# romz-pl/linear-programming-Vanderbei

Hardware: AMD Instinct MI355X
Metric: IPM iterations/sec (ADA^T factor+solve) on netlib dfl001; duality gap ≤1e-8 (higher is better)
Workload: dtype f64; 1 GPU; dfl001 hsd (BASELINE configs[2]), one step = one complete solve to mu < 1e-12; method=hsd, m=12155, n=12230, nz=71277, parallelism=replicas1, status=optimal solution, lnz=7160813, nsup=18147, levels=20, refine_passes=251

## Files before the change

### linear-programming-vanderbei_amd/csrc/dev_common.h

```cpp
#pragma once
#include <hip/hip_runtime.h>

#include <vector>

#include "row_ax.h"

namespace ipo {

constexpr int kRedBlocks = 256;
constexpr int kRedThreads = 256;

__device__ __forceinline__ double ref_max(double x, double y) { return x > y ? x : y; }
__device__ __forceinline__ double ref_abs(double x) { return x > 0 ? x : -x; }

template <int N>
__device__ __forceinline__ double dpp_row_down(double v) {
    const long long b = __double_as_longlong(v);
    const int lo = (int)b, hi = (int)(b >> 32);
    const int lo2 = __builtin_amdgcn_update_dpp(lo, lo, 0x100 + N, 0xf, 0xf, false);
    const int hi2 = __builtin_amdgcn_update_dpp(hi, hi, 0x100 + N, 0xf, 0xf, false);
    return __longlong_as_double(((long long)hi2 << 32) | (unsigned int)lo2);
}

__device__ __forceinline__ double wave_sum(double v) {
    v += __shfl_down(v, 32, 64);
    v += __shfl_down(v, 16, 64);
    v += dpp_row_down<8>(v);
    v += dpp_row_down<4>(v);
    v += dpp_row_down<2>(v);
    v += dpp_row_down<1>(v);
    return v;
}
__device__ __forceinline__ double wave_max(double v) {
    v = fmax(v, __shfl_down(v, 32, 64));
    v = fmax(v, __shfl_down(v, 16, 64));
    v = fmax(v, dpp_row_down<8>(v));
    v = fmax(v, dpp_row_down<4>(v));
    v = fmax(v, dpp_row_down<2>(v));
    v = fmax(v, dpp_row_down<1>(v));
    return v;
}

__device__ __forceinline__ double sparse_dot(int kb, int ke, const double* __restrict__ v, const int* __restrict__ idx,
                                             const double* __restrict__ x) {
    double s = 0.0;
    int k = kb;
    for (; k + 16 <= ke; k += 16) {
        int ix[16];
        double a[16], b[16];
#pragma unroll
        for (int u = 0; u < 16; u++) { ix[u] = idx[k + u]; a[u] = v[k + u]; }
#pragma unroll
        for (int u = 0; u < 16; u++) b[u] = x[ix[u]];
#pragma unroll
        for (int u = 0; u < 16; u++) s += a[u] * b[u];
    }
    const int rem = ke - k;
    if (rem > 0) {
        int ix[16];
        double a[16], b[16];
#pragma unroll
        for (int u = 0; u < 16; u++)
            if (u < rem) { ix[u] = idx[k + u]; a[u] = v[k + u]; }
#pragma unroll
        for (int u = 0; u < 16; u++)
            if (u < rem) b[u] = x[ix[u]];
#pragma unroll
        for (int u = 0; u < 16; u++)
            if (u < rem) s += a[u] * b[u];
    }
    return s;
}

template <int NW>
__device__ __forceinline__ double block_sum_w(double v, double* sh ) {
    v = wave_sum(v);
    const int lane = threadIdx.x & 63, w = threadIdx.x >> 6;
    if (lane == 0) sh[w] = v;
    __syncthreads();
    double r = 0.0;
    if (threadIdx.x == 0) {
        r = sh[0];
#pragma unroll
        for (int q = 1; q < NW; q++) r += sh[q];
    }
    __syncthreads();
    return r;
}
template <int NW>
__device__ __forceinline__ double block_max_w(double v, double* sh) {
    v = wave_max(v);
    const int lane = threadIdx.x & 63, w = threadIdx.x >> 6;
    if (lane == 0) sh[w] = v;
    __syncthreads();
    double r = 0.0;
    if (threadIdx.x == 0) {
        r = sh[0];
#pragma unroll
        for (int q = 1; q < NW; q++) r = fmax(r, sh[q]);
    }
    __syncthreads();
    return r;
}
constexpr int kResThreads = 1024;

__device__ __forceinline__ double block_sum(double v, double* sh ) {
    v = wave_sum(v);
    const int lane = threadIdx.x & 63, w = threadIdx.x >> 6;
    if (lane == 0) sh[w] = v;
    __syncthreads();
    double r = 0.0;
    if (threadIdx.x == 0) r = (sh[0] + sh[1]) + (sh[2] + sh[3]);
    __syncthreads();
    return r;
}
__device__ __forceinline__ double block_max(double v, double* sh) {
    v = wave_max(v);
    const int lane = threadIdx.x & 63, w = threadIdx.x >> 6;
    if (lane == 0) sh[w] = v;
    __syncthreads();
    double r = 0.0;
    if (threadIdx.x == 0) r = fmax(fmax(sh[0], sh[1]), fmax(sh[2], sh[3]));
    __syncthreads();
    return r;
}

__global__ void __launch_bounds__(kRedThreads)
k_finish_reduce(const double* __restrict__ part, int nq, unsigned maxmask, double* __restrict__ out);
__global__ void __launch_bounds__(kRedThreads)
k_finish_reduce_pack(const double* __restrict__ part, int nq, unsigned maxmask, double* __restrict__ out,
                     const int* __restrict__ f, int nf, double* __restrict__ outi);

struct RedJobs {
    const double* a[8];
    const double* b[8];
    int len[8];
    int op[8];
    int nj;
    int segmin;
};
__global__ void __launch_bounds__(kRedThreads)
k_reduce_jobs(RedJobs jobs, double* __restrict__ part);

constexpr int kOrderedMaxLen = 1 << 19;
constexpr int kSegDotLen = 1 << 12;
constexpr int kSegMaxLen = 1 << 16;
__host__ __device__ inline int dot_segmin(const RedJobs& j) { return j.segmin > 0 ? j.segmin : kOrderedMaxLen; }
__host__ __device__ inline bool job_segmented(const RedJobs& j, int q) {
    return j.len[q] >= (j.op[q] == 0 ? dot_segmin(j) : kSegMaxLen);
}
extern bool g_ordered_reductions;
void launch_reduce(const RedJobs& jobs, double* part, double* out, hipStream_t st);
double dot_ordered_host(const double* a, const double* b, int n);

void launch_link_ax(int mrow, int m, const int* kAt, const int* iAt, const double* At, const double* x, double* out,
                    hipStream_t st);

void launch_q_long(int nl, const int* cols, const int* kQ, const int* iQ, const double* Q, const double* v,
                   double* out, hipStream_t st);
__host__ __device__ inline bool q_col_long(const int* kQ, int j, int thr) {
    return thr > 0 && kQ[j + 1] - kQ[j] >= thr;
}
std::vector<int> q_long_columns(int n, const int* kQ, int thr);
void q_times_host(int n, const int* kQ, const int* iQ, const double* Q, const double* v, int thr, double* out);

}
```

### linear-programming-vanderbei_amd/csrc/dev_common.hip

```cpp
#include "dev_common.h"

#include <algorithm>
#include <cstdlib>
#include <stdexcept>
#include <vector>
#include "hip_util.h"

namespace ipo {

__global__ void __launch_bounds__(kRedThreads)
k_reduce_jobs(RedJobs jobs, double* __restrict__ part) {
    __shared__ double sh[4];
    for (int j = 0; j < jobs.nj; j++) {
        const double* a = jobs.a[j];
        const double* b = jobs.b[j];
        const int len = jobs.len[j];
        const int op = jobs.op[j];
        double acc = op == 0 ? 0.0 : (op == 2 ? 0.0 : 0.0);
        for (int i = blockIdx.x * kRedThreads + threadIdx.x; i < len; i += kRedBlocks * kRedThreads) {
            if (op == 0) acc += a[i] * b[i];
            else if (op == 1) acc = fmax(acc, ref_abs(a[i]));
            else acc = fmax(acc, -a[i] / b[i]);
        }
        const double r = op == 0 ? block_sum(acc, sh) : block_max(acc, sh);
        if (threadIdx.x == 0) part[j * kRedBlocks + blockIdx.x] = r;
    }
}

__global__ void __launch_bounds__(kRedThreads)
k_finish_reduce(const double* __restrict__ part, int nq, unsigned maxmask, double* __restrict__ out) {
    __shared__ double sh[4];
    for (int q = 0; q < nq; q++) {
        const bool mx = (maxmask >> q) & 1u;
        double v = part[q * kRedBlocks + threadIdx.x];
        const double r = mx ? block_max(v, sh) : block_sum(v, sh);
        if (threadIdx.x == 0) out[q] = r;
    }
}

__global__ void __launch_bounds__(kRedThreads)
k_finish_reduce_pack(const double* __restrict__ part, int nq, unsigned maxmask, double* __restrict__ out,
                     const int* __restrict__ f, int nf, double* __restrict__ outi) {
    __shared__ double sh[4];
    for (int q = 0; q < nq; q++) {
        const bool mx = (maxmask >> q) & 1u;
        double v = part[q * kRedBlocks + threadIdx.x];
        const double r = mx ? block_max(v, sh) : block_sum(v, sh);
        if (threadIdx.x == 0) out[q] = r;
    }
    if (static_cast<int>(threadIdx.x) < nf) reinterpret_cast<int*>(outi)[threadIdx.x] = f[threadIdx.x];
}

constexpr int kOrdThreads = 256;

__global__ void __launch_bounds__(kOrdThreads)
k_reduce_ordered(RedJobs jobs, double* __restrict__ out) {
    const int j = blockIdx.x;
    const double* a = jobs.a[j];
    const double* b = jobs.b[j];
    const int len = jobs.len[j];
    const int op = jobs.op[j];
    const int tid = threadIdx.x;
    if (job_segmented(jobs, j)) return;
    if (op != 0) {
        __shared__ double sh[4];
        double acc = 0.0;
        for (int i0 = 0; i0 < len; i0 += 8 * kOrdThreads) {
            double va[8], vb[8];
#pragma unroll
            for (int u = 0; u < 8; u++) {
                const int i = i0 + u * kOrdThreads + tid;
                va[u] = i < len ? a[i] : 0.0;
                vb[u] = op == 2 && i < len ? b[i] : 1.0;
            }
#pragma unroll
            for (int u = 0; u < 8; u++) {
                if (i0 + u * kOrdThreads + tid >= len) continue;
                if (op == 1) acc = fmax(acc, ref_abs(va[u]));
                else acc = fmax(acc, -va[u] / vb[u]);
            }
        }
        acc = block_max(acc, sh);
        if (tid == 0) out[j] = acc;
        return;
    }
    constexpr int CH = 4096;
    __shared__ __attribute__((aligned(16))) double comp[2][CH + 16];
    __shared__ int nzc[2], ready[2], freed[2];
    if (tid < 2) {
        ready[tid] = 0;
        freed[tid] = 0;
    }
    __syncthreads();
    const int nch = (len + CH - 1) / CH, lane = tid & 63, wv = tid >> 6;
    if (wv == 1) {
        for (int k = 0; k < nch; k++) {
            const int buf = k & 1;
            if (k >= 2)
                while (__hip_atomic_load(&freed[buf], __ATOMIC_ACQUIRE, __HIP_MEMORY_SCOPE_WORKGROUP) < k - 1)
                    __builtin_amdgcn_s_sleep(1);
            const int base = k * CH, cnt = min(CH, len - base);
            int off = 0;
            for (int i0 = 0; i0 < cnt; i0 += 8 * 64) {
                double pa[8], pb[8];
#pragma unroll
                for (int u = 0; u < 8; u++) {
                    const int i = i0 + u * 64 + lane;
                    pa[u] = i < cnt ? a[base + i] : 0.0;
                    pb[u] = i < cnt ? b[base + i] : 0.0;
                }
#pragma unroll
                for (int u = 0; u < 8; u++) {
                    const double v = pa[u] * pb[u];
                    const bool nzf = i0 + u * 64 + lane < cnt && v != 0.0;
                    const unsigned long long m = __ballot(nzf);
                    if (nzf) comp[buf][off + __popcll(m & ((1ull << lane) - 1ull))] = v;
                    off += __popcll(m);
                }
            }
            if (lane == 0) {
                nzc[buf] = off;
                __hip_atomic_store(&ready[buf], k + 1, __ATOMIC_RELEASE, __HIP_MEMORY_SCOPE_WORKGROUP);
            }
        }
        return;
    }
    if (tid != 0) return;
    double s = 0.0e0;
    for (int k = 0; k < nch; k++) {
        const int buf = k & 1;
        while (__hip_atomic_load(&ready[buf], __ATOMIC_ACQUIRE, __HIP_MEMORY_SCOPE_WORKGROUP) < k + 1)
            __builtin_amdgcn_s_sleep(1);
        const int nz = nzc[buf];
        const double2* pp = reinterpret_cast<const double2*>(comp[buf]);
        double2 cur[8];
#pragma unroll
        for (int u = 0; u < 8; u++) cur[u] = pp[u];
        int i = 0;
        for (; i + 16 <= nz; i += 16) {
            double2 nxt[8];
#pragma unroll
            for (int u = 0; u < 8; u++) nxt[u] = pp[(i + 16) / 2 + u];
#pragma unroll
            for (int u = 0; u < 8; u++) { s += cur[u].x; s += cur[u].y; }
#pragma unroll
            for (int u = 0; u < 8; u++) cur[u] = nxt[u];
        }
        for (; i < nz; i++) s += comp[buf][i];
        __hip_atomic_store(&freed[buf], k + 1, __ATOMIC_RELEASE, __HIP_MEMORY_SCOPE_WORKGROUP);
    }
    out[j] = s;
}

double dot_ordered_host(const double* a, const double* b, int n) {
    DevBuf<double> da(std::max(1, n)), db(std::max(1, n)), dout(8), dpart(8 * kRedBlocks);
    IPO_HIP_CHECK(hipMemcpy(da.get(), a, n * sizeof(double), hipMemcpyHostToDevice));
    IPO_HIP_CHECK(hipMemcpy(db.get(), b, n * sizeof(double), hipMemcpyHostToDevice));
    RedJobs j{};
    j.nj = 1;
    j.a[0] = da.get(); j.b[0] = db.get(); j.len[0] = n; j.op[0] = 0;
    launch_reduce(j, dpart.get(), dout.get(), nullptr);
    double r = 0.0;
    IPO_HIP_CHECK(hipMemcpy(&r, dout.get(), sizeof(double), hipMemcpyDeviceToHost));
    return r;
}

__global__ void __launch_bounds__(kOrdThreads)
k_dot_segments(RedJobs jobs, double* __restrict__ part) {
    const int j = blockIdx.y, g = blockIdx.x, tid = threadIdx.x;
    const int len = jobs.len[j], op = jobs.op[j];
    if (!job_segmented(jobs, j)) return;
    const long seg = (static_cast<long>(len) + kRedBlocks - 1) / kRedBlocks;
    const long b = seg * g, e = min(static_cast<long>(len), b + seg);
    const double* a = jobs.a[j];
    const double* bb = jobs.b[j];
    __shared__ double sh[kOrdThreads];
    double acc = 0.0;
    for (long i0 = b; i0 < e; i0 += 8 * kOrdThreads) {
        double pa[8], pb[8];
#pragma unroll
        for (int u = 0; u < 8; u++) {
            const long i = i0 + u * kOrdThreads + tid;
            pa[u] = i < e ? a[i] : 0.0;
            pb[u] = i < e && op != 1 ? bb[i] : 1.0;
        }
#pragma unroll
        for (int u = 0; u < 8; u++) {
            if (i0 + u * kOrdThreads + tid >= e) continue;
            if (op == 0) acc += pa[u] * pb[u];
            else if (op == 1) acc = fmax(acc, ref_abs(pa[u]));
            else acc = fmax(acc, -pa[u] / pb[u]);
        }
    }
    sh[tid] = acc;
    __syncthreads();
    if (tid == 0) {
        double s = 0.0;
        for (int t = 0; t < kOrdThreads; t++) s = op == 0 ? s + sh[t] : fmax(s, sh[t]);
        part[j * kRedBlocks + g] = s;
    }
}

__global__ void __launch_bounds__(64)
k_dot_finish(RedJobs jobs, const double* __restrict__ part, double* __restrict__ out) {
    const int j = threadIdx.x;
    if (j >= jobs.nj || !job_segmented(jobs, j)) return;
    const bool mx = jobs.op[j] != 0;
    double s = 0.0;
    for (int g = 0; g < kRedBlocks; g++) s = mx ? fmax(s, part[j * kRedBlocks + g]) : s + part[j * kRedBlocks + g];
    out[j] = s;
}

__global__ void __launch_bounds__(256)
k_link_ax(int mrow, int m, const int* __restrict__ kAt, const int* __restrict__ iAt, const double* __restrict__ At,
          const double* __restrict__ x, double* __restrict__ out) {
    const int i = mrow + blockIdx.x * 4 + (threadIdx.x >> 6), lane = threadIdx.x & 63;
    if (i >= m) return;
    double s = 0.0;
    for (int k = kAt[i] + lane; k < kAt[i + 1]; k += 64) s += At[k] * x[iAt[k]];
    s = wave_sum(s);
    if (lane == 0) out[i - mrow] = s;
}

void launch_link_ax(int mrow, int m, const int* kAt, const int* iAt, const double* At, const double* x, double* out,
                    hipStream_t st) {
    if (m <= mrow) return;
    hipLaunchKernelGGL(k_link_ax, dim3((m - mrow + 3) / 4), dim3(256), 0, st, mrow, m, kAt, iAt, At, x, out);
    IPO_HIP_CHECK(hipGetLastError());
}

constexpr int kQLongSteps = 4;

__global__ void __launch_bounds__(256)
k_q_long(int nl, const int* __restrict__ cols, const int* __restrict__ kQ, const int* __restrict__ iQ,
// ... 106 lines not shown
        for (int u = 0; u < 8; u++)
            if (ok[u]) b[u] = x[c[u]];
#pragma unroll
        for (int u = 0; u < 8; u++)
            if (ok[u]) s += a[u] * b[u];
    }
    ax[i] = s;
}

bool rows_ax_sliced(const KktKnobs& knobs, int n) {
    if (knobs.ax_jds >= 0) return knobs.ax_jds != 0;
    return knobs.ax_blocks > 1 || static_cast<long>(n) * static_cast<long>(sizeof(double)) > kAxSliceBytes;
}

void RowAxPlan::build(int m, int n, const int* kA, const int* iA, const double* A, int npass, hipStream_t st) {
    m_ = m;
    np_ = std::max(1, npass);
    const int per = (n + np_ - 1) / np_;
    auto slice = [&](int j) { return per > 0 ? std::min(np_ - 1, j / per) : 0; };
    std::vector<int> cnt(static_cast<size_t>(np_) * m, 0);
    for (int j = 0; j < n; j++)
        for (int k = kA[j]; k < kA[j + 1]; k++) cnt[static_cast<size_t>(slice(j)) * m + iA[k]]++;
    std::vector<int> perm(static_cast<size_t>(np_) * m), rank(static_cast<size_t>(np_) * m), dptr, dlen;
    rows_.assign(np_, 0);
    nd_.assign(np_, 0);
    dbase_.assign(np_ + 1, 0);
    long nz = 0;
    for (int p = 0; p < np_; p++) {
        const int* c = cnt.data() + static_cast<size_t>(p) * m;
        int mx = 0;
        for (int i = 0; i < m; i++) mx = std::max(mx, c[i]);
        std::vector<int> bucket(mx + 2, 0);
        for (int i = 0; i < m; i++) bucket[mx - c[i] + 1]++;
        for (int v = 0; v <= mx; v++) bucket[v + 1] += bucket[v];
        int* pp = perm.data() + static_cast<size_t>(p) * m;
        int* rk = rank.data() + static_cast<size_t>(p) * m;
        for (int i = 0; i < m; i++) { const int r = bucket[mx - c[i]]++; pp[r] = i; rk[i] = r; }
        int active = 0;
        while (active < m && c[pp[active]] > 0) active++;
        rows_[p] = p == 0 ? m : active;
        nd_[p] = mx;
        for (int k = 0, len = active; k < mx; k++) {
            while (len > 0 && c[pp[len - 1]] <= k) len--;
            dptr.push_back(static_cast<int>(nz));
            dlen.push_back(len);
            nz += len;
        }
        dbase_[p + 1] = static_cast<int>(dptr.size());
    }
    if (nz > static_cast<long>(INT32_MAX)) throw std::length_error("row products: more than 2^31 entries");
    std::vector<int> cols(nz), fill(static_cast<size_t>(np_) * m, 0);
    std::vector<double> vals(nz);
    for (int j = 0; j < n; j++) {
        const int p = slice(j);
        for (int k = kA[j]; k < kA[j + 1]; k++) {
            const size_t pi = static_cast<size_t>(p) * m + iA[k];
            const int q = dptr[dbase_[p] + fill[pi]++] + rank[pi];
            cols[q] = j;
            vals[q] = A[k];
        }
    }
    perm_.upload(perm, st);
    dptr_.upload(dptr, st);
    dlen_.upload(dlen, st);
    cols_.upload(cols, st);
    vals_.upload(vals, st);
    IPO_HIP_CHECK(hipStreamSynchronize(st));
}

void RowAxPlan::launch(const double* x, double* ax, hipStream_t st) const {
    for (int p = 0; p < np_; p++) {
        if (rows_[p] <= 0) continue;
        hipLaunchKernelGGL(k_rows_ax_jds, dim3((rows_[p] + 255) / 256), dim3(256), 0, st, rows_[p],
                           perm_.get() + static_cast<size_t>(p) * m_, dptr_.get() + dbase_[p], dlen_.get() + dbase_[p],
                           nd_[p], cols_.get(), vals_.get(), x, p == 0 ? 1 : 0, ax);
    }
    IPO_HIP_CHECK(hipGetLastError());
}

bool g_ordered_reductions = true;

void launch_reduce(const RedJobs& jobs, double* part, double* out, hipStream_t st) {
    if (g_ordered_reductions) {
        hipLaunchKernelGGL(k_reduce_ordered, dim3(jobs.nj), dim3(kOrdThreads), 0, st, jobs, out);
        bool longdot = false;
        for (int j = 0; j < jobs.nj; j++) longdot |= job_segmented(jobs, j);
        if (longdot) {
            hipLaunchKernelGGL(k_dot_segments, dim3(kRedBlocks, jobs.nj), dim3(kOrdThreads), 0, st, jobs, part);
            hipLaunchKernelGGL(k_dot_finish, dim3(1), dim3(64), 0, st, jobs, part, out);
        }
        IPO_HIP_CHECK(hipGetLastError());
        return;
    }
    unsigned mask = 0;
    for (int j = 0; j < jobs.nj; j++) if (jobs.op[j] != 0) mask |= 1u << j;
    hipLaunchKernelGGL(k_reduce_jobs, dim3(kRedBlocks), dim3(kRedThreads), 0, st, jobs, part);
    hipLaunchKernelGGL(k_finish_reduce, dim3(1), dim3(kRedThreads), 0, st, part, jobs.nj, mask, out);
    IPO_HIP_CHECK(hipGetLastError());
}

}
```

### linear-programming-vanderbei_amd/csrc/ipm.h

```cpp
#pragma once
#include <hip/hip_runtime.h>

#include <cstdio>
#include <memory>

#include "exchange.h"
#include "hip_util.h"
#include "kkt_device.h"
#include "row_ax.h"

namespace ipo {

enum class Method { Hsd = 0, Intpt = 1, Hsdls = 2, Qp = 3, Pc = 4 };

struct IpmOptions {
    Method method = Method::Hsd;
    int max_iter = 200;
    FILE* trace = nullptr;
    bool timing = false;
};

struct IpmResult {
    int status = 5;
    int iters = 0;
    double t_setup_s = 0.0;
    double t_solve_s = 0.0;
    double final_mu = 0.0, final_pobj = 0.0, final_dobj = 0.0, final_pinf = 0.0, final_dinf = 0.0;
    double phi = 1.0, psi = 1.0;
    KktTimers kkt;
    long refine_passes = 0;
};

struct ShardSpec {
    int nforced = 0;
    Exchange* xch = nullptr;
    int m_global = 0, n_global = 0;
    long nz_global = 0;
};

constexpr int kIsRed = 0;
constexpr int kIsZx = 0, kIsWy = 1, kIsCx = 2, kIsBy = 3;
constexpr int kIsXqx = 4;
constexpr int kIsPhiMu = 6;
constexpr int kIsNorm2 = 8;
constexpr int kIsTheta = 11;
constexpr int kIsDphi = 12;
constexpr int kIsPhiNext = 14;
constexpr int kIsPcRatio = 16;
constexpr int kIsPcDots = 17;
constexpr int kIsPcMu = 23;
constexpr int kIsCount = 24;

void vector_bench(int m, int n, const int* kA, const int* iA, const double* A, int reps, double* out, double* bytes);

class IpmSolver {
  public:
    IpmSolver(int m, int n, const int* kA, const int* iA, const double* A, const double* b, const double* c,
              double f, hipStream_t stream = nullptr, const ShardSpec* shard = nullptr, const QBlock* q = nullptr);
    ~IpmSolver();
    int run(const IpmOptions& opt, IpmResult* res);
    void download(double* x, double* y, double* w, double* z) const;
    KktDevice& kkt() { return *kkt_; }
    double setup_seconds() const { return t_setup_; }

  private:
    int run_hsd(const IpmOptions& opt, IpmResult* res);
    int run_intpt(const IpmOptions& opt, IpmResult* res);
    int run_hsdls(const IpmOptions& opt, IpmResult* res);
    int run_qp(const IpmOptions& opt, IpmResult* res);
    template <bool SW>
    int run_pc(const IpmOptions& opt, IpmResult* res);
    void reduce(const struct RedJobs& j, int nout);
    void link_ax(const double* x);
    void xsum(double* d, size_t n, RedOp op) { if (xch_) xch_->allreduce(d, n, op, stream_); }
    const double* lax() const { return xch_ ? lax_.get() : axsliced_ ? ax_.get() : nullptr; }
    int mrow() const { return xch_ ? m_ - nforced_ : axsliced_ ? 0 : m_; }
    void row_ax(const double* x, hipStream_t st);
    const KktKnobs knobs_ = KktKnobs::from_env();
    bool axsliced_ = false;
    DevBuf<double> ax_;
    RowAxPlan axplan_;
    void print_dims(FILE* tr) const;

    int m_, n_;
    double f_;
    hipStream_t stream_;
    bool own_stream_ = false;
    double t_setup_ = 0.0;
    int nforced_ = 0;
    Exchange* xch_ = nullptr;
    int mcnt_ = 0;
    int mg_ = 0, ng_ = 0;
    int dot_segmin_ = 0;
    long nzg_ = 0;
    std::unique_ptr<KktDevice> kkt_;
    bool has_q_ = false, sharded_ = false;
    DevBuf<double> qx_;
    DevBuf<double> b_, c_, x_, y_, w_, z_;
    DevBuf<double> rho_, sig_, D_, E_, fx_, fy_, gx_, gy_, dx_, dy_, dz_, dw_;
    DevBuf<double> part_, part2_, scal_, lax_;
    hipStream_t side_ = nullptr;
    hipEvent_t ev_step_ = nullptr, ev_side_ = nullptr;
    double* hs_ = nullptr;
};

int ipm_solve_host(int m, int n, int nz, const int* iA, const int* kA, const double* A, const double* b,
                   const double* c, double f, double* x, double* y, double* w, double* z, const IpmOptions& opt,
                   IpmResult* res);

}
```

### linear-programming-vanderbei_amd/csrc/ipm_device.hip

```cpp
#include <hip/hip_runtime.h>

#include <chrono>
#include <cmath>
#include <cstdlib>
#include <cstring>
#include <exception>
#include <stdexcept>
#include <vector>

#include "dev_common.h"
#include "hip_util.h"
#include "ipm.h"
#include "lp_io.h"

namespace ipo {

namespace {

constexpr int NT = 256;

__global__ void __launch_bounds__(NT) k_fill(int n, double v, double* __restrict__ a) {
    const int i = blockIdx.x * NT + threadIdx.x;
    if (i < n) a[i] = v;
}

__global__ void __launch_bounds__(kResThreads)
k_hsd_residuals(int m, int n, const int* __restrict__ kAt, const int* __restrict__ iAt, const double* __restrict__ At,
                const int* __restrict__ kA, const int* __restrict__ iA, const double* __restrict__ A,
                const double* __restrict__ b, const double* __restrict__ c, const double* __restrict__ x,
                const double* __restrict__ y, const double* __restrict__ w, const double* __restrict__ z, double phi_h,
                double delta, double mu_h, double* __restrict__ E, double* __restrict__ D, double* __restrict__ fy,
                double* __restrict__ fx, double* __restrict__ gy, double* __restrict__ gx, double* __restrict__ part,
                int mrow, int mcnt, const double* __restrict__ lax, const double* __restrict__ phimu) {
    __shared__ double sh[kResThreads / 64];
    const double phi = phimu ? phimu[0] : phi_h;
    const double mu = phimu ? phimu[1] : mu_h;
    const bool wde = phimu == nullptr;
    double sr = 0.0, ss = 0.0;
    for (int i = blockIdx.x * kResThreads + threadIdx.x; i < m + n; i += kRedBlocks * kResThreads) {
        if (i < m) {
            double ax = 0.0;
            if (i >= mrow) ax = lax[i - mrow];
            else
                ax = sparse_dot(kAt[i], kAt[i + 1], At, iAt, x);
            const double r1 = ax - b[i] * phi + w[i];
            if (i < mcnt) sr += r1 * r1;
            const double rho = -(1 - delta) * r1 + w[i] - delta * mu / y[i];
            if (wde) E[i] = w[i] / y[i];
            fy[i] = rho;
            gy[i] = -b[i];
        } else {
            const int j = i - m;
            double aty = 0.0;
            aty = sparse_dot(kA[j], kA[j + 1], A, iA, y);
            const double s1 = -aty + c[j] * phi + z[j];
            ss += s1 * s1;
            const double sg = -(1 - delta) * s1 + z[j] - delta * mu / x[j];
            if (wde) D[j] = z[j] / x[j];
            fx[j] = -sg;
            gx[j] = -c[j];
        }
    }
    sr = block_sum_w<kResThreads / 64>(sr, sh);
    ss = block_sum_w<kResThreads / 64>(ss, sh);
    if (threadIdx.x == 0) { part[blockIdx.x] = sr; part[kRedBlocks + blockIdx.x] = ss; }
}

__global__ void __launch_bounds__(NT)
k_hsd_directions(int m, int n, const double* __restrict__ dphip, double delta, double mu, const double* __restrict__ fx,
                 const double* __restrict__ gx, const double* __restrict__ fy, const double* __restrict__ gy,
                 const double* __restrict__ x, const double* __restrict__ z, const double* __restrict__ y,
                 const double* __restrict__ w, const double* __restrict__ D, const double* __restrict__ E,
                 double* __restrict__ dx, double* __restrict__ dz, double* __restrict__ dy, double* __restrict__ dw,
                 double* __restrict__ part) {
    __shared__ double sh[4];
    const double dphi = *dphip;
    double th = 0.0;
    for (int i = blockIdx.x * NT + threadIdx.x; i < m + n; i += kRedBlocks * NT) {
        if (i < n) {
            const double ddx = fx[i] - gx[i] * dphi;
            const double ddz = delta * mu / x[i] - z[i] - D[i] * ddx;
            dx[i] = ddx; dz[i] = ddz;
            th = fmax(th, -ddx / x[i]);
            th = fmax(th, -ddz / z[i]);
        } else {
            const int j = i - n;
            const double ddy = fy[j] - gy[j] * dphi;
            const double ddw = delta * mu / y[j] - w[j] - E[j] * ddy;
            dy[j] = ddy; dw[j] = ddw;
            th = fmax(th, -ddy / y[j]);
            th = fmax(th, -ddw / w[j]);
        }
    }
    th = block_max(th, sh);
    if (threadIdx.x == 0) part[blockIdx.x] = th;
}

__global__ void __launch_bounds__(NT)
k_step(int m, int n, double theta_h, const double* __restrict__ thetap, double* __restrict__ x,
       const double* __restrict__ dx, double* __restrict__ z, const double* __restrict__ dz, double* __restrict__ y,
       const double* __restrict__ dy, double* __restrict__ w, const double* __restrict__ dw) {
    const double theta = thetap ? *thetap : theta_h;
    const int i = blockIdx.x * NT + threadIdx.x;
    if (i < n) { x[i] = x[i] + theta * dx[i]; z[i] = z[i] + theta * dz[i]; }
    else if (i < n + m) { const int j = i - n; y[j] = y[j] + theta * dy[j]; w[j] = w[j] + theta * dw[j]; }
}

__global__ void __launch_bounds__(NT)
k_hsd_scaling(int m, int n, const double* __restrict__ x, const double* __restrict__ y, const double* __restrict__ w,
              const double* __restrict__ z, double* __restrict__ E, double* __restrict__ D) {
    const int i = blockIdx.x * NT + threadIdx.x;
    if (i < m) E[i] = w[i] / y[i];
    else if (i < m + n) { const int j = i - m; D[j] = z[j] / x[j]; }
}

__global__ void k_hsd_mu(double* sc, double denom, double phi_h, double psi_h, int dev) {
    const double phi = dev ? sc[kIsPhiNext] : phi_h, psi = dev ? sc[kIsPhiNext + 1] : psi_h;
    sc[kIsPhiMu] = phi;
    sc[kIsPhiMu + 1] = (sc[kIsZx] + sc[kIsWy] + phi * psi) / denom;
}

__global__ void k_hsd_dphi(double* sc, double gamma, double delta, double mu, double phi, double psi) {
    const double* red = sc + kIsRed;
    const double dphi = (red[0] - red[1] + gamma) / (red[2] - red[3] - psi / phi);
    const double dpsi = delta * mu / phi - psi - (psi / phi) * dphi;
    sc[kIsDphi] = dphi;
    sc[kIsDphi + 1] = dpsi;
}

__global__ void k_hsd_theta(double* sc, double phi, double psi) {
    const double dphi = sc[kIsDphi], dpsi = sc[kIsDphi + 1];
    double theta = sc[kIsRed];
    if (theta < -dphi / phi) theta = -dphi / phi;
    if (theta < -dpsi / psi) theta = -dpsi / psi;
    theta = (0.95 / theta > 1.0) ? 1.0 : 0.95 / theta;
    sc[kIsTheta] = theta;
    sc[kIsPhiNext] = phi + theta * dphi;
    sc[kIsPhiNext + 1] = psi + theta * dpsi;
}

__global__ void __launch_bounds__(NT)
k_unscale(int m, int n, double phi, double* __restrict__ x, double* __restrict__ z, double* __restrict__ y,
          double* __restrict__ w) {
    const int i = blockIdx.x * NT + threadIdx.x;
    if (i < n) { x[i] /= phi; z[i] /= phi; }
    else if (i < n + m) { const int j = i - n; y[j] /= phi; w[j] /= phi; }
}

__device__ __forceinline__ double ls_step(double xj, double zj, double dxj, double dzj, double beta, double delta,
                                          double mu) {
    const double a = dxj * dzj;
    const double b = zj * dxj + xj * dzj + (1 - beta) * (1 - delta) * mu;
    const double c = xj * zj - (1 - beta) * mu;
    const double d = b * b - 4 * a * c;
    if (a == 0.0) return -c / b;
    if (a > 0) {
        if (b < 0) {
            if (d >= 0) return 2 * c / (-b + sqrt(d));
            return HUGE_VAL;
        }
        return HUGE_VAL;
    }
    if (b < 0) return 2 * c / (-b + sqrt(d));
    return (-b - sqrt(d)) / (2 * a);
}

__global__ void __launch_bounds__(NT)
k_hsdls_directions(int m, int n, double dphi, double beta, double delta, double mu, const double* __restrict__ fx,
                   const double* __restrict__ gx, const double* __restrict__ fy, const double* __restrict__ gy,
                   const double* __restrict__ x, const double* __restrict__ z, const double* __restrict__ y,
                   const double* __restrict__ w, const double* __restrict__ D, const double* __restrict__ E,
                   double* __restrict__ dx, double* __restrict__ dz, double* __restrict__ dy, double* __restrict__ dw,
                   double* __restrict__ part) {
    __shared__ double sh[4];
    double th = -HUGE_VAL;
    for (int i = blockIdx.x * NT + threadIdx.x; i < m + n; i += kRedBlocks * NT) {
        if (i < n) {
            const double ddx = fx[i] - gx[i] * dphi;
            const double ddz = delta * mu / x[i] - z[i] - D[i] * ddx;
            dx[i] = ddx; dz[i] = ddz;
            th = fmax(th, -ls_step(x[i], z[i], ddx, ddz, beta, delta, mu));
        } else {
            const int j = i - n;
            const double ddy = fy[j] - gy[j] * dphi;
            const double ddw = delta * mu / y[j] - w[j] - E[j] * ddy;
            dy[j] = ddy; dw[j] = ddw;
            th = fmax(th, -ls_step(y[j], w[j], ddy, ddw, beta, delta, mu));
        }
    }
    th = block_max(th, sh);
    if (threadIdx.x == 0) part[blockIdx.x] = th;
}

__global__ void __launch_bounds__(kResThreads)
k_pf_residuals(int m, int n, const int* __restrict__ kAt, const int* __restrict__ iAt, const double* __restrict__ At,
               const int* __restrict__ kA, const int* __restrict__ iA, const double* __restrict__ A,
               const double* __restrict__ b, const double* __restrict__ c, const double* __restrict__ x,
               const double* __restrict__ y, const double* __restrict__ w, const double* __restrict__ z,
               double* __restrict__ rho, double* __restrict__ sig, double* __restrict__ part, int mrow, int mcnt,
               const double* __restrict__ lax) {
    __shared__ double sh[kResThreads / 64];
    double sr = 0.0, ss = 0.0;
    for (int i = blockIdx.x * kResThreads + threadIdx.x; i < m + n; i += kRedBlocks * kResThreads) {
        if (i < m) {
            double ax = 0.0;
            if (i >= mrow) ax = lax[i - mrow];
            else
                ax = sparse_dot(kAt[i], kAt[i + 1], At, iAt, x);
            const double r = b[i] - ax - w[i];
            rho[i] = r;
            if (i < mcnt) sr += r * r;
        } else {
            const int j = i - m;
            double aty = 0.0;
            aty = sparse_dot(kA[j], kA[j + 1], A, iA, y);
            const double s = c[j] - aty + z[j];
            sig[j] = s;
            ss += s * s;
        }
    }
    sr = block_sum_w<kResThreads / 64>(sr, sh);
// ... 208 lines not shown
    const double a = dxj * dzj;
    const double b = zj * dxj + xj * dzj + (1 - beta) * (1 - delta) * mu;
    const double c = xj * zj - (1 - beta) * mu;
    const double d = b * b - 4 * a * c;
    if (a == 0.0) return -c / b;
    if (a > 0) return (b < 0 && d >= 0) ? 2 * c / (-b + std::sqrt(d)) : HUGE_VAL;
    if (b < 0) return 2 * c / (-b + std::sqrt(d));
    return (-b - std::sqrt(d)) / (2 * a);
}

double now_s() {
    return std::chrono::duration<double>(std::chrono::steady_clock::now().time_since_epoch()).count();
}

const char* kHsdHeader =
    "--------------------------------------------------------------------------\n"
    "         |           Primal          |            Dual           |       |\n"
    "  Iter   |  Obj Value       Infeas   |  Obj Value       Infeas   |  mu   |\n"
    "- - - - - - - - - - - - - - - - - - - - - - - - - - - - - - - - - - - - - \n";
const char* kIntptHeader =
    "------------------------------------------------------------------\n"
    "         |           Primal          |            Dual           |\n"
    "  Iter   |  Obj Value       Infeas   |  Obj Value       Infeas   |\n"
    "- - - - - - - - - - - - - - - - - - - - - - - - - - - - - - - - - \n";

}

IpmSolver::IpmSolver(int m, int n, const int* kA, const int* iA, const double* A, const double* b, const double* c,
                     double f, hipStream_t stream, const ShardSpec* shard, const QBlock* q)
    : m_(m), n_(n), f_(f), stream_(stream) {
    const double t0 = now_s();
    sharded_ = shard != nullptr;
    has_q_ = q && q->kQ && q->kQ[n] > 0;
    if (has_q_ && sharded_) throw std::invalid_argument("qp: a solver with Q cannot be sharded");
    mg_ = m;
    ng_ = n;
    nzg_ = kA[n];
    mcnt_ = m;
    if (shard) {
        if (shard->nforced < 0 || shard->nforced > m) throw std::invalid_argument("shard: nforced out of range");
        nforced_ = shard->nforced;
        xch_ = shard->xch;
        if (xch_) {
            mg_ = shard->m_global;
            ng_ = shard->n_global;
            nzg_ = shard->nz_global;
            if (xch_->rank() != 0) mcnt_ = m - nforced_;
        }
    }
    dot_segmin_ = knobs_.dot_segmin >= 0 ? knobs_.dot_segmin : std::max(mg_, ng_) >= kOrderedMaxLen ? kSegDotLen : 0;
    if (!stream_) {
        IPO_HIP_CHECK(hipStreamCreateWithFlags(&stream_, hipStreamNonBlocking));
        own_stream_ = true;
    }
    if (has_q_) {
        std::vector<int> kat, iat;
        std::vector<double> at;
        csc_transpose(m, n, kA, iA, A, kat, iat, at);
        QBlock qb = *q;
        qb.qmax = 1;
        kkt_ = std::make_unique<KktDevice>(n, m, kat.data(), iat.data(), at.data(), stream_, 0, &qb);
    } else {
        kkt_ = std::make_unique<KktDevice>(m, n, kA, iA, A, stream_, nforced_);
        kkt_->set_exchange(xch_);
    }
    if (dot_segmin_ > 0 && !xch_ && !has_q_) {
        constexpr int kLongRow = 256;
        std::vector<int> cnt(m > 0 ? m : 1, 0);
        for (int k = 0; k < kA[n]; k++) cnt[iA[k]]++;
        int r0 = m;
        while (r0 > 0 && cnt[r0 - 1] >= kLongRow) r0--;
        if (r0 < m) kkt_->set_long_rows(r0);
    }
    const size_t mm = m > 0 ? m : 1, nn = n > 0 ? n : 1;
    b_.upload(b, m, stream_);
    c_.upload(c, n, stream_);
    for (DevBuf<double>* v : {&x_, &z_, &sig_, &D_, &fx_, &gx_, &dx_, &dz_, &qx_}) v->alloc(nn);
    for (DevBuf<double>* v : {&y_, &w_, &rho_, &E_, &fy_, &gy_, &dy_, &dw_}) v->alloc(mm);
    if (m == 0) b_.alloc(1);
    if (n == 0) c_.alloc(1);
    part_.alloc(8 * kRedBlocks);
    part2_.alloc(8 * kRedBlocks);
    scal_.alloc(kIsCount);
    IPO_HIP_CHECK(hipStreamCreateWithFlags(&side_, hipStreamNonBlocking));
    IPO_HIP_CHECK(hipEventCreateWithFlags(&ev_step_, hipEventDisableTiming));
    IPO_HIP_CHECK(hipEventCreateWithFlags(&ev_side_, hipEventDisableTiming));
    lax_.alloc(nforced_ > 0 ? nforced_ : 1);
    axsliced_ = rows_ax_sliced(knobs_, n_) && !xch_;
    if (axsliced_) {
        ax_.alloc(m_ > 0 ? m_ : 1);
        axplan_.build(m, n, kA, iA, A, knobs_.ax_blocks, stream_);
    }
    IPO_HIP_CHECK(hipHostMalloc(reinterpret_cast<void**>(&hs_), kIsCount * sizeof(double), hipHostMallocDefault));
    IPO_HIP_CHECK(hipStreamSynchronize(stream_));
    t_setup_ = now_s() - t0;
}

IpmSolver::~IpmSolver() {
    if (side_) (void)hipStreamSynchronize(side_);
    if (hs_) (void)hipHostFree(hs_);
    if (ev_step_) (void)hipEventDestroy(ev_step_);
    if (ev_side_) (void)hipEventDestroy(ev_side_);
    if (side_) (void)hipStreamDestroy(side_);
    kkt_.reset();
    if (own_stream_) (void)hipStreamDestroy(stream_);
}

void IpmSolver::reduce(const RedJobs& j, int nout) {
    launch_reduce(j, part_.get(), scal_.get(), stream_);
    xsum(scal_.get(), nout, RedOp::Sum);
    IPO_HIP_CHECK(hipMemcpyAsync(hs_, scal_.get(), nout * sizeof(double), hipMemcpyDeviceToHost, stream_));
    IPO_HIP_CHECK(hipStreamSynchronize(stream_));
}

void IpmSolver::row_ax(const double* x, hipStream_t st) {
    if (!axsliced_) return;
    axplan_.launch(x, ax_.get(), st);
}

void IpmSolver::link_ax(const double* x) {
    row_ax(x, stream_);
    if (!xch_ || nforced_ == 0) return;
    launch_link_ax(m_ - nforced_, m_, kkt_->kAt(), kkt_->iAt(), kkt_->At(), x, lax_.get(), stream_);
    xsum(lax_.get(), nforced_, RedOp::Sum);
}

void IpmSolver::print_dims(FILE* tr) const { std::fprintf(tr, "m = %d,n = %d,nz = %ld\n", mg_, ng_, nzg_); }

void IpmSolver::download(double* x, double* y, double* w, double* z) const {
    if (x) x_.download(x, n_, stream_);
    if (y) y_.download(y, m_, stream_);
    if (w) w_.download(w, m_, stream_);
    if (z) z_.download(z, n_, stream_);
    IPO_HIP_CHECK(hipStreamSynchronize(stream_));
}

int IpmSolver::run(const IpmOptions& opt, IpmResult* res) {
    IpmResult local;
    if (!res) res = &local;
    *res = IpmResult();
    const bool qp = opt.method == Method::Qp;
    if (qp && sharded_) throw std::invalid_argument("qp: not supported on a sharded solver");
    const bool pc = opt.method == Method::Pc;
    if (pc && sharded_) throw std::invalid_argument("pc: not supported on a sharded solver");
    if (!qp && !pc && has_q_) throw std::invalid_argument("a solver built with Q runs method qp only (hsd, intpt and hsdls are LP methods)");
    KktDevice& K = *kkt_;
    res->t_setup_s = t_setup_;
    K.enable_timing(opt.timing);
    K.reset_timers();
    K.set_epsdiag(1.0e-14);
    const double t0 = now_s();
    const int st = qp                            ? (has_q_ ? run_qp(opt, res) : run_intpt(opt, res))
                   : pc                          ? (has_q_ ? run_pc<true>(opt, res) : run_pc<false>(opt, res))
                   : opt.method == Method::Intpt ? run_intpt(opt, res)
                   : opt.method == Method::Hsdls ? run_hsdls(opt, res)
                                                 : run_hsd(opt, res);
    res->t_solve_s = now_s() - t0;
    res->status = st;
    res->kkt = K.timers();
    return st;
}

int IpmSolver::run_hsd(const IpmOptions& opt, IpmResult* res) {
    const bool overlap = xch_ == nullptr && knobs_.overlap;
    const int m = m_, n = n_;
    hipStream_t s = stream_;
    const int gv = ceil_div(m + n, NT);
    FILE* tr = opt.trace;
    hipLaunchKernelGGL(k_fill, dim3(ceil_div(n, NT)), dim3(NT), 0, s, n, 1.0, x_.get());
    hipLaunchKernelGGL(k_fill, dim3(ceil_div(n, NT)), dim3(NT), 0, s, n, 1.0, z_.get());
    hipLaunchKernelGGL(k_fill, dim3(ceil_div(m, NT)), dim3(NT), 0, s, m, 1.0, w_.get());
    hipLaunchKernelGGL(k_fill, dim3(ceil_div(m, NT)), dim3(NT), 0, s, m, 1.0, y_.get());
    double phi = 1.0, psi = 1.0;
    if (tr) {
        print_dims(tr);
        std::fputs(kHsdHeader, tr);
        std::fflush(tr);
    }
    KktDevice& K = *kkt_;
    int status = 5, iter;
    for (iter = 0; iter < opt.max_iter; iter++) {
        RedJobs j{};
        j.nj = 4;
        j.segmin = dot_segmin_;
        j.a[0] = z_.get(); j.b[0] = x_.get(); j.len[0] = n; j.op[0] = 0;
        j.a[1] = w_.get(); j.b[1] = y_.get(); j.len[1] = mcnt_; j.op[1] = 0;
        j.a[2] = c_.get(); j.b[2] = x_.get(); j.len[2] = n; j.op[2] = 0;
        j.a[3] = b_.get(); j.b[3] = y_.get(); j.len[3] = mcnt_; j.op[3] = 0;
        const double delta = (iter % 2 == 0) ? 0.0 : 1.0;
        KktDevice::HostState spec{};
        std::exception_ptr spec_err;
        if (overlap) {
            IPO_HIP_CHECK(hipEventRecord(ev_step_, s));
            IPO_HIP_CHECK(hipStreamWaitEvent(side_, ev_step_, 0));
            launch_reduce(j, part2_.get(), scal_.get(), side_);
            hipLaunchKernelGGL(k_hsd_mu, dim3(1), dim3(1), 0, side_, scal_.get(), static_cast<double>(ng_ + mg_ + 1), phi,
                               psi, iter > 0 ? 1 : 0);
            row_ax(x_.get(), side_);
            hipLaunchKernelGGL(k_hsd_residuals, dim3(kRedBlocks), dim3(kResThreads), 0, side_, m, n, K.kAt(), K.iAt(),
                               K.At(), K.kA(), K.iA(), K.A(), b_.get(), c_.get(), x_.get(), y_.get(), w_.get(), z_.get(),
                               phi, delta, 0.0, E_.get(), D_.get(), fy_.get(), fx_.get(), gy_.get(), gx_.get(),
                               part2_.get(), mrow(), mcnt_, lax(), static_cast<const double*>(scal_.get() + kIsPhiMu));
            hipLaunchKernelGGL(k_finish_reduce, dim3(1), dim3(kRedThreads), 0, side_, part2_.get(), 2, 0u,
                               scal_.get() + kIsNorm2);
            IPO_HIP_CHECK(hipMemcpyAsync(hs_, scal_.get(), kIsCount * sizeof(double), hipMemcpyDeviceToHost, side_));
            IPO_HIP_CHECK(hipEventRecord(ev_side_, side_));
            hipLaunchKernelGGL(k_hsd_scaling, dim3(gv), dim3(NT), 0, s, m, n, x_.get(), y_.get(), w_.get(), z_.get(),
                               E_.get(), D_.get());
            spec = K.host_state();
            KktDevice::PrePass pre;
            pre.R = 2;
            pre.dfy[0] = fy_.get(); pre.dfx[0] = fx_.get();
            pre.dfy[1] = gy_.get(); pre.dfx[1] = gx_.get();
            pre.stream = side_;
            pre.ready = ev_side_;
            try {
                K.factor(E_.get(), D_.get(), &pre);
            } catch (...) {
                spec_err = std::current_exception();
            }
            IPO_HIP_CHECK(hipEventSynchronize(ev_side_));
        } else {
            launch_reduce(j, part_.get(), scal_.get(), s);
            xsum(scal_.get(), 4, RedOp::Sum);
            IPO_HIP_CHECK(hipMemcpyAsync(hs_, scal_.get(), 4 * sizeof(double), hipMemcpyDeviceToHost, s));
            if (iter > 0)
                IPO_HIP_CHECK(hipMemcpyAsync(hs_ + kIsPhiNext, scal_.get() + kIsPhiNext, 2 * sizeof(double),
                                             hipMemcpyDeviceToHost, s));
            IPO_HIP_CHECK(hipStreamSynchronize(s));
        }
        if (iter > 0) { phi = hs_[kIsPhiNext]; psi = hs_[kIsPhiNext + 1]; }
        const double mu = (hs_[kIsZx] + hs_[kIsWy] + phi * psi) / (ng_ + mg_ + 1);
        if (overlap && (std::memcmp(&mu, &hs_[kIsPhiMu + 1], sizeof mu) != 0 ||
                        std::memcmp(&phi, &hs_[kIsPhiMu], sizeof phi) != 0))
            throw std::runtime_error("hsd: device mu / phi differ from the host's");
        const double pobj = hs_[kIsCx], dobj = hs_[kIsBy];
        if (mu < 1.0e-12) {
            if (overlap) K.restore_host_state(spec);
            if (phi > psi) status = 0;
            else if (dobj < 0.0) status = 2;
            else if (pobj > 0.0) status = 4;
            else { if (tr) std::fprintf(tr, "Trouble in river city \n"); status = 4; }
            break;
        }
        if (!overlap) {
            link_ax(x_.get());
            hipLaunchKernelGGL(k_hsd_residuals, dim3(kRedBlocks), dim3(kResThreads), 0, s, m, n, K.kAt(), K.iAt(), K.At(),
                               K.kA(), K.iA(), K.A(), b_.get(), c_.get(), x_.get(), y_.get(), w_.get(), z_.get(), phi,
                               delta, mu, E_.get(), D_.get(), fy_.get(), fx_.get(), gy_.get(), gx_.get(), part_.get(),
                               mrow(), mcnt_, lax(), static_cast<const double*>(nullptr));
            hipLaunchKernelGGL(k_finish_reduce, dim3(1), dim3(kRedThreads), 0, s, part_.get(), 2, 0u, scal_.get());
            xsum(scal_.get(), 2, RedOp::Sum);
            IPO_HIP_CHECK(hipMemcpyAsync(hs_ + kIsNorm2, scal_.get() + kIsRed, 2 * sizeof(double),
                                         hipMemcpyDeviceToHost, s));
            K.factor(E_.get(), D_.get());
        } else {
            if (spec_err) std::rethrow_exception(spec_err);
            IPO_HIP_CHECK(hipStreamWaitEvent(s, ev_side_, 0));
        }
        const double gamma = -(1 - delta) * (dobj - pobj + psi) + psi - delta * mu / phi;

        const double normr = std::sqrt(hs_[kIsNorm2]) / phi;
        const double norms = std::sqrt(hs_[kIsNorm2 + 1]) / phi;
        if (tr) {
            std::fprintf(tr, "%8d   %14.7e  %8.1e    %14.7e  %8.1e  %8.1e \n", iter, pobj / phi + f_, normr,
                         dobj / phi + f_, norms, mu);
            std::fflush(tr);
        }
        res->final_mu = mu; res->final_pobj = pobj / phi + f_; res->final_dobj = dobj / phi + f_;
        res->final_pinf = normr; res->final_dinf = norms;
        if (knobs_.trace_full) {
            std::fprintf(stderr, "FT %d %.17g %.17g %.17g %.17g %.17g %.17g\n", iter, pobj, dobj, mu, phi, psi, normr);
            std::fprintf(stderr, "FT   ndep=%d eps=%.1e\n", K.ndep(), K.epsdiag());
        }
        K.solve2(E_.get(), D_.get(), fy_.get(), fx_.get(), gy_.get(), gx_.get());
        res->refine_passes += K.last_passes();

        RedJobs q{};
        q.nj = 4;
        q.segmin = dot_segmin_;
        q.a[0] = c_.get(); q.b[0] = fx_.get(); q.len[0] = n; q.op[0] = 0;
        q.a[1] = b_.get(); q.b[1] = fy_.get(); q.len[1] = mcnt_; q.op[1] = 0;
        q.a[2] = c_.get(); q.b[2] = gx_.get(); q.len[2] = n; q.op[2] = 0;
        q.a[3] = b_.get(); q.b[3] = gy_.get(); q.len[3] = mcnt_; q.op[3] = 0;
        launch_reduce(q, part_.get(), scal_.get(), s);
        xsum(scal_.get(), 4, RedOp::Sum);
        hipLaunchKernelGGL(k_hsd_dphi, dim3(1), dim3(1), 0, s, scal_.get(), gamma, delta, mu, phi, psi);
        hipLaunchKernelGGL(k_hsd_directions, dim3(kRedBlocks), dim3(NT), 0, s, m, n, scal_.get() + kIsDphi, delta, mu,
                           fx_.get(), gx_.get(), fy_.get(), gy_.get(), x_.get(), z_.get(), y_.get(), w_.get(), D_.get(),
                           E_.get(), dx_.get(), dz_.get(), dy_.get(), dw_.get(), part_.get());
        hipLaunchKernelGGL(k_finish_reduce, dim3(1), dim3(kRedThreads), 0, s, part_.get(), 1, 1u, scal_.get());
        xsum(scal_.get(), 1, RedOp::Max);
        hipLaunchKernelGGL(k_hsd_theta, dim3(1), dim3(1), 0, s, scal_.get(), phi, psi);
        hipLaunchKernelGGL(k_step, dim3(gv), dim3(NT), 0, s, m, n, 0.0, scal_.get() + kIsTheta, x_.get(), dx_.get(),
                           z_.get(), dz_.get(), y_.get(), dy_.get(), w_.get(), dw_.get());
    }
    hipLaunchKernelGGL(k_unscale, dim3(gv), dim3(NT), 0, s, m, n, phi, x_.get(), z_.get(), y_.get(), w_.get());
    IPO_HIP_CHECK(hipGetLastError());
    IPO_HIP_CHECK(hipStreamSynchronize(s));
    res->iters = iter;
    res->phi = phi;
    res->psi = psi;
    return status;
}

int IpmSolver::run_hsdls(const IpmOptions& opt, IpmResult* res) {
    const int m = m_, n = n_;
    hipStream_t s = stream_;
    const int gv = ceil_div(m + n, NT);
    FILE* tr = opt.trace;
    hipLaunchKernelGGL(k_fill, dim3(ceil_div(n, NT)), dim3(NT), 0, s, n, 1.0, x_.get());
    hipLaunchKernelGGL(k_fill, dim3(ceil_div(n, NT)), dim3(NT), 0, s, n, 1.0, z_.get());
    hipLaunchKernelGGL(k_fill, dim3(ceil_div(m, NT)), dim3(NT), 0, s, m, 1.0, w_.get());
    hipLaunchKernelGGL(k_fill, dim3(ceil_div(m, NT)), dim3(NT), 0, s, m, 1.0, y_.get());
    double phi = 1.0, psi = 1.0;
    if (tr) {
        print_dims(tr);
        std::fputs(kHsdHeader, tr);
        std::fflush(tr);
    }
    const double beta = 0.80, delta = 2 * (1 - beta);
    KktDevice& K = *kkt_;
    int status = 5, iter;
    for (iter = 0; iter < opt.max_iter; iter++) {
        RedJobs j{};
        j.nj = 4;
        j.segmin = dot_segmin_;
        j.a[0] = z_.get(); j.b[0] = x_.get(); j.len[0] = n; j.op[0] = 0;
        j.a[1] = w_.get(); j.b[1] = y_.get(); j.len[1] = mcnt_; j.op[1] = 0;
        j.a[2] = c_.get(); j.b[2] = x_.get(); j.len[2] = n; j.op[2] = 0;
        j.a[3] = b_.get(); j.b[3] = y_.get(); j.len[3] = mcnt_; j.op[3] = 0;
        reduce(j, 4);
        const double mu = (hs_[kIsZx] + hs_[kIsWy] + phi * psi) / (ng_ + mg_ + 1);
        const double pobj = hs_[kIsCx], dobj = hs_[kIsBy];
        if (mu < 1.0e-12) {
            if (phi > 1.0e-12) status = 0;
            else if (dobj < 0.0) status = 2;
            else if (pobj > 0.0) status = 4;
            else status = 7;
            break;
        }
        link_ax(x_.get());
        hipLaunchKernelGGL(k_hsd_residuals, dim3(kRedBlocks), dim3(kResThreads), 0, s, m, n, K.kAt(), K.iAt(), K.At(), K.kA(),
                           K.iA(), K.A(), b_.get(), c_.get(), x_.get(), y_.get(), w_.get(), z_.get(), phi, delta, mu,
                           E_.get(), D_.get(), fy_.get(), fx_.get(), gy_.get(), gx_.get(), part_.get(), mrow(), mcnt_,
                           lax(), static_cast<const double*>(nullptr));
        hipLaunchKernelGGL(k_finish_reduce, dim3(1), dim3(kRedThreads), 0, s, part_.get(), 2, 0u, scal_.get());
        xsum(scal_.get(), 2, RedOp::Sum);
        IPO_HIP_CHECK(hipMemcpyAsync(hs_, scal_.get(), 2 * sizeof(double), hipMemcpyDeviceToHost, s));
        IPO_HIP_CHECK(hipStreamSynchronize(s));
        const double normr = std::sqrt(hs_[kIsRed]) / phi;
        const double norms = std::sqrt(hs_[kIsRed + 1]) / phi;
        const double gamma = -(1 - delta) * (dobj - pobj + psi) + psi - delta * mu / phi;
        if (tr) {
            std::fprintf(tr, "%8d   %14.7e  %8.1e    %14.7e  %8.1e  %8.1e \n", iter, pobj / phi + f_, normr,
                         dobj / phi + f_, norms, mu);
            std::fflush(tr);
        }
        res->final_mu = mu; res->final_pobj = pobj / phi + f_; res->final_dobj = dobj / phi + f_;
        res->final_pinf = normr; res->final_dinf = norms;

        K.factor(E_.get(), D_.get());
        K.solve2(E_.get(), D_.get(), fy_.get(), fx_.get(), gy_.get(), gx_.get());
        res->refine_passes += K.last_passes();

        RedJobs q{};
        q.nj = 4;
        q.segmin = dot_segmin_;
        q.a[0] = c_.get(); q.b[0] = fx_.get(); q.len[0] = n; q.op[0] = 0;
        q.a[1] = b_.get(); q.b[1] = fy_.get(); q.len[1] = mcnt_; q.op[1] = 0;
        q.a[2] = c_.get(); q.b[2] = gx_.get(); q.len[2] = n; q.op[2] = 0;
        q.a[3] = b_.get(); q.b[3] = gy_.get(); q.len[3] = mcnt_; q.op[3] = 0;
        reduce(q, 4);
        const double dphi = (hs_[kIsRed] - hs_[kIsRed + 1] + gamma) / (hs_[kIsRed + 2] - hs_[kIsRed + 3] - psi / phi);
        const double dpsi = delta * mu / phi - psi - (psi / phi) * dphi;

        hipLaunchKernelGGL(k_hsdls_directions, dim3(kRedBlocks), dim3(NT), 0, s, m, n, dphi, beta, delta, mu, fx_.get(),
                           gx_.get(), fy_.get(), gy_.get(), x_.get(), z_.get(), y_.get(), w_.get(), D_.get(), E_.get(),
// ... 369 lines not shown
```

### linear-programming-vanderbei_amd/csrc/kkt_device.h

```cpp
#pragma once
#include <hip/hip_runtime.h>

#include <cstddef>
#include <cstdint>
#include <memory>
#include <vector>

#include "hip_util.h"
#include "exchange.h"
#include "kkt_flags.h"
#include "kkt_knobs.h"
#include "kkt_plan.h"
#include "kkt_schedule.h"

namespace ipo {

struct TailView {
    double* S;
    int nt, ntb, tc;
    const int* task_ptr;
    const TailTask* tasks;
    double* W;
    int vk = kTailVisitBlocks;
    int dep = 1;
// ... 33 lines not shown
static_assert(RunCounters::vseq_at(3) == 4 && RunCounters::pread_at(3) == 13 && RunCounters::cdone_at(3) == 16 &&
                  RunCounters::lead_ticket_at(3) == 19 && RunCounters::words(3) == 20,
              "run counters, ntb = 3: 1 + 3 + 9 + 3 + 3 + 1");

constexpr int kTailPubWin = 16 * 64 + 16;

struct ChainGran {
    static constexpr size_t kZ = 2 * 64 * 2;
    static constexpr size_t kPart = 2 * 4 * 64 * 2;
    static constexpr size_t part_at(size_t ntb) { return ntb * kZ; }
    static constexpr size_t words(size_t ntb) { return ntb * (kZ + kPart); }
};

struct KktTimers {
    double phase_ms[kNumPhases] = {};
    long phase_launches[kNumPhases] = {};
    long phase_count[kNumPhases] = {};
    double factor_ms = 0.0;
    double solve_ms = 0.0;
    double sweep_ms = 0.0;
    long factors = 0, solves = 0, rawsolves = 0;
    long panel_redos = 0;
    long redo_where[4] = {0, 0, 0, 0};
    long tail_repairs = 0;
    long tail_dep_rounds = 0;
};

constexpr int kScRes = 0;
constexpr int kScEps = 4;
constexpr int kScIncons = 6;
constexpr int kScReadLater = kScIncons + 1;
constexpr int kScMaxbc = 8;
constexpr int kScCount = kScMaxbc + 4;
constexpr int kFsNegMinD = 0;
constexpr int kFsNdepMax = 1;
constexpr int kFsBailMax = 2;
constexpr int kFsFlags = 3;
constexpr int kFsCount = kFsFlags + 2;

struct QBlock {
    const int* kQ = nullptr;
    const int* iQ = nullptr;
    const double* Q = nullptr;
    int qmax = 1;
};

struct PlanView;

class KktDevice {
  public:
    KktDevice(int m, int n, const int* kA, const int* iA, const double* A, hipStream_t stream, int nforced = 0,
              const QBlock* qb = nullptr);
    ~KktDevice();
    KktDevice(const KktDevice&) = delete;
    KktDevice& operator=(const KktDevice&) = delete;

    const KktPlan& plan() const { return plan_; }
    void set_exchange(Exchange* x) { xch_ = x; }
    int nforced() const { return nforced_; }
    int m() const { return m_; }
    int n() const { return n_; }
    hipStream_t stream() const { return stream_; }

    const int* kA() const { return dkA_.get(); }
    const int* iA() const { return diA_.get(); }
    const double* A() const { return dA_.get(); }
    const int* kAt() const { return dkAt_.get(); }
    const int* iAt() const { return diAt_.get(); }
    const double* At() const { return dAt_.get(); }
    const int* kQ() const { return qnz_ > 0 ? dkQ_.get() : nullptr; }
    const int* iQ() const { return qnz_ > 0 ? diQ_.get() : nullptr; }
    const double* Q() const { return qnz_ > 0 ? dQ_.get() : nullptr; }
    int q_long_count() const { return q_long_n_; }
    int q_long_min() const { return q_long_n_ > 0 ? knobs_.q_long : 0; }
    void launch_q_long(const double* v, double* out);

    struct PrePass {
        int R = 0;
        double* dfy[2] = {nullptr, nullptr};
        double* dfx[2] = {nullptr, nullptr};
        hipStream_t stream = nullptr;
        hipEvent_t ready = nullptr;
    };
    void factor(const double* dE, const double* dD, const PrePass* pre = nullptr);
    int solve(const double* dE, const double* dD, double* dfy, double* dfx);
    int solve2(const double* dE, const double* dD, double* dfy1, double* dfx1, double* dfy2, double* dfx2);
    void solve_multi(int R, const double* dE, const double* dD, double* const* dfy, double* const* dfx, int* ok);

    void rawsolve(double* dz, int R = 1, size_t fwd_first = 0);

    struct HostState {
        double epsdiag;
        int ndep;
        KktTimers tm;
    };
    HostState host_state() const { return {epsdiag_, ndep_, tm_}; }
    void restore_host_state(const HostState& h) { epsdiag_ = h.epsdiag; ndep_ = h.ndep; tm_ = h.tm; drop_prepass(); }

    double epsdiag() const { return epsdiag_; }
    void set_pivot_tolerance(double t) { pivot_tol_ = t; }
    void set_epsdiag(double e) { epsdiag_ = e; }
    void set_long_rows(int row0);
    double pivot_tolerance() const { return pivot_tol_; }
    int ndep() const { return ndep_; }
    int last_passes() const { return last_passes_; }
    const KktTimers& timers() const { return tm_; }
    void enable_timing(bool on) { timing_ = on; }
    void reset_timers() { tm_ = KktTimers(); }

    void download_factor(double* lx, double* d, int* live = nullptr) const;
    double* device_lx() const { return dLx_.get(); }
    double* device_diag() const { return dDg_.get(); }

  private:
    const KktKnobs knobs_ = KktKnobs::from_env();
    void upload_plan(const int* kA, const int* iA, const double* A, const std::vector<int>& kat,
                     const std::vector<int>& iat, const std::vector<double>& at, const QBlock* qb);
    void build_panel_units();
    SolveChunks build_solve_chunks();
    SweepOrder build_sweep_order(const SolveChunks& ch);
    void build_sync_free_plan(const SolveChunks& ch, const SweepOrder& so, int cus);
    void build_gather_chunks(const VisitSlots& vs);
    void count_work();
    void build_slot_records(const std::vector<int>& kslot_v);
    void setup_tail(int cus);
    void alloc_numeric();
    void raise_sweep_lds(bool sync_free);
    void dump_sf_stamps() const;
    KktLaunch h_;
    PlanView plan_view() const;
    bool tail_repair() const { return use_panel_ && !xch_ && knobs_.tail_repair; }
    void factor_core(const double* dE, const double* dD, const PrePass* pre);
    void dump_factor(const double* dE, const double* dD, double eps_in);
    int dump_count_ = 0;
    TailView tail_view() const;
    template <int R>
    void sweep(double* dz, const double* epsp, size_t fwd_first);
    template <int R>
    int run_sweep_steps(const std::vector<SweepStep>& steps, bool forward, double* dz, const double* epsp,
                        size_t first = 0, size_t last = SIZE_MAX, hipStream_t s = nullptr);
    void tail_rhs_begin(double* dz, int R);
    void tail_rhs_end(double* dz, int R);
    DevBuf<int> dIncons_;
    int launch_gather(const struct PlanView& pv, const TailView& tv, int tail, int group, hipStream_t s);
    void launch_reduce_maxabs2(const double* a, int na, const double* b, int nb, double* dst);

    int m_, n_, T_;
    int nforced_ = 0;
    Exchange* xch_ = nullptr;
    DevBuf<double> dLinkAx_;
    int long_row0_ = -1;
    DevBuf<double> dLongAx_;
    bool shard_minor() const { return xch_ && xch_->rank() != 0; }
    void xsum(double* d, size_t n, RedOp op) { if (xch_) xch_->allreduce(d, n, op, stream_); }
    hipStream_t stream_;
    KktPlan plan_;
    double epsdiag_ = 1.0e-14;
    int ndep_ = 0;
    double pivot_tol_ = knobs_.pivtol;
    int last_passes_ = 0;
    bool timing_ = false;
    KktTimers tm_;
    hipEvent_t ev0_ = nullptr, ev1_ = nullptr, ev2_ = nullptr, ev3_ = nullptr;
    std::vector<hipEvent_t> kev_;
    size_t kev_used_ = 0;
    struct PhaseMark { hipEvent_t b, e; int phase, launches; };
    std::vector<PhaseMark> marks_;
    hipEvent_t mark_b_ = nullptr;
    hipEvent_t next_event();
    void ph_begin(hipStream_t s);
    void ph_end(int phase, int launches, hipStream_t s);
    void ph_collect();
  public:
    double work_flops[kNumPhases] = {}, work_bytes[kNumPhases] = {};
  private:

    DevBuf<int> dkA_, diA_, dkAt_, diAt_;
    DevBuf<double> dA_, dAt_;
    int qnz_ = 0, qmax_ = 1;
    DevBuf<int> dkQ_, diQ_;
    DevBuf<double> dQ_, dQdiag_;
    DevBuf<int64_t> dqmap_;
    int q_long_n_ = 0;
    DevBuf<int> dQLongCols_;
    DevBuf<double> dLongQ_;
    DevBuf<int> dcol0_, drowptr_, drows_, dperm_, diperm_;
    DevBuf<int64_t> doff_, damap_, ddslot_, drelptr_;
    DevBuf<int> dunit_sup_, dunit_tile_, dtask_ptr_, dtask_pair_, dtask_i0_, dtask_i1_;
    DevBuf<int> dupd_src_, dupd_r0_, dupd_r1_, drel_, dlevel_sups_;
    DevBuf<int> dyrow_ptr_, dyrow_idx_;
    DevBuf<int> dylate_ptr_, dylate_idx_, dpre_col_, dpre_ptr_, dpre_idx_;
    DevBuf<double> dYbuf_;
    int sf_grid_ = 1;
    int sf_fwd_epoch_ = 0, sf_bwd_epoch_ = 0;
    long long sf_ticket_next_[2] = {0, 0};
#ifdef IPO_SF_STAMPS
    std::vector<SchedInt2> h_sf_items_f_;
#endif
    int sf_tbase(int d, int nitems, hipStream_t s);
    DevBuf<int2> dsf_items_f_, dsf_items_b_;
    DevBuf<int> dsf_need_, dsf_par_, dsf_zbase_, dsf_zpi_, dsf_fcnt_, dsf_fflag_, dsf_bcnt_, dsf_bflag_, dsf_ticket_;
    DevBuf<int> dybase_;
    DevBuf<double> dZpad_;
    DevBuf<int> dfu_sup_, dfu_j_;
    DevBuf<int> dsmall_sups_;
    const bool use_panel_ = knobs_.panel;
    bool factor_pass(const double* dE, const double* dD, bool fused, bool tail_fused, const PrePass* pre = nullptr);
    bool prepass_eligible(const PrePass* pre, bool fused, bool tail_fused) const;
    void enqueue_prepass(const PrePass& pre);
    void run_prepass_steps(int R, hipStream_t q);
    void enqueue_pass_head(int R, double* const* dfy, double* const* dfx, double* part, hipStream_t s);
    bool take_prepass(int R, double* const* dfy, double* const* dfx);
    void drop_prepass() {
        if (pre_state_ != kPreNone) { pre_state_ = kPreNone; pre_discarded_++; lead_discarded_ += pre_lead_; }
        pre_lead_ = false;
        lead_pending_ = 0;
    }
    enum { kPreNone = 0, kPreEnqueued, kPreValid };
    int pre_state_ = kPreNone;
    PrePass pre_req_;
    hipEvent_t ev_pre_fork_ = nullptr, ev_pre_done_ = nullptr;
    long pre_used_ = 0, pre_discarded_ = 0;
    int lead_pending_ = 0;
    bool pre_lead_ = false;
    hipEvent_t ev_run_reset_ = nullptr;
    long lead_used_ = 0, lead_discarded_ = 0;
    void launch_lead_trail(int R, hipStream_t s, bool beside);
    DevBuf<double> dPrePart_;
    void enqueue_levels(const PlanView& pv, const TailView& tv, bool fused, hipStream_t s, const PrePass* pre);
    bool finish_pass(bool fused);
    void repair_tail();
    DevBuf<int> dsweep_sups_;
    DevBuf<int> dchunk_sup_, dchunk_r0_, dsup_chunk0_;
    DevBuf<double> dPartial_;
    int gst_group_ = knobs_.gather_stamps, gst_n_ = 0;
    DevBuf<long long> dGStamp_;
    DevBuf<int> dck_u_, dck_b_, dck_e_, dck_part_, dsp_u_, dsp_p0_, dsp_n_;
    DevBuf<int> dck_q_;
    DevBuf<int> dSplitCnt_;
    bool eps_cleared_ = false;
    DevBuf<double> dPartialTile_;
    DevBuf<TaskSrc> dusrc_, dtsrc_;
    DevBuf<SlotRec> dslot_rec_, dtail_slot_rec_;
    DevBuf<unsigned long long> dChainGran_;
    int chain_epoch_ = 0;
    DevBuf<int> dtail_task_ptr_, dtail_kslot_, dtail_kslot_ptr_;
    DevBuf<int> dlead_ticket_;
    long long lead_ticket_next_ = 0;
    DevBuf<unsigned> dvisit_list_;
    DevBuf<uint2> drun_items_;
    DevBuf<int> drun_cnt_;
    RunCounters run_counters() const { return RunCounters(drun_cnt_.get(), plan_.ntb); }
    DevBuf<double> drun_pub_;
    DevBuf<int> drun_wflag_;
    int run_epoch_ = 0;
    void launch_tail_from(int t0, bool reset);
    DevBuf<uint64_t> dtail_tasks_, dutasks_;
    DevBuf<double> dW_;
    DevBuf<double> dDepSt_;
    DevBuf<int> dDepI_;
    DevBuf<double> dLx_, dDg_;
    DevBuf<int> dLive_;
    DevBuf<double> dDscale_;
    DevBuf<int> dFlags_;
    DevBuf<int> dSign_;
    DevBuf<double> dZ_, dDy_, dDx_, dRy_, dRx_;
    DevBuf<double> dPart_;
    DevBuf<double> dScal_;
    double* sweep_eps() const { return dScal_.get() + kScEps; }
    DevBuf<double> dFacScal_;
    double* hScal_ = nullptr;
    int* hDepDone_ = nullptr;
    FactorVerdict verdict_;
};

}
```

### linear-programming-vanderbei_amd/csrc/kkt_device.hip

```cpp
#include <hip/hip_runtime.h>

#include <chrono>
#include <algorithm>
#include <cmath>
#include <cstdio>
#include <cstdlib>
#include <cstring>

#include "dev_common.h"
#include "kkt_device.h"
#include "kkt_kernels.h"
#include "lp_io.h"

namespace ipo {

namespace {

__global__ void __launch_bounds__(NT)
k_assemble_A(int nz, const double* __restrict__ A, const int64_t* __restrict__ amap, double* __restrict__ Lx) {
    const int k = blockIdx.x * NT + threadIdx.x;
    if (k < nz) Lx[amap[k]] = A[k];
}

__global__ void __launch_bounds__(NT)
k_assemble_Q(int nq, const double* __restrict__ Q, const int64_t* __restrict__ qmap, double qmax,
             double* __restrict__ Lx) {
    const int k = blockIdx.x * NT + threadIdx.x;
    if (k < nq && qmap[k] >= 0) Lx[qmap[k]] = -qmax * Q[k];
}

__global__ void __launch_bounds__(NT)
k_assemble_diag(int T, int m, const int* __restrict__ perm, const double* __restrict__ E,
                const double* __restrict__ D, double eps, const int64_t* __restrict__ dslot,
                double* __restrict__ Lx, int* __restrict__ live, double* __restrict__ dscale, int tail_from,
                int* __restrict__ flags, const double* __restrict__ qdiag, double qmax) {
    const int v = blockIdx.x * NT + threadIdx.x;
    if (v < kFlagWords) flags[v] = 0;
    if (v >= T) return;
    const int old = perm[v];
    double a = v >= tail_from ? 0.0 : old < m ? -ref_max(E[old], eps) : ref_max(D[old - m], eps);
    double sc = fabs(a);
    if (qdiag && old < m) {
        const double q = qmax * qdiag[old];
        a = a - q;
        sc = sc + fabs(q);
    }
    Lx[dslot[v]] = a;
    dscale[v] = sc;
    live[v] = 1;
}

__global__ void __launch_bounds__(NT) k_zero_tail_lower(double* __restrict__ S, int nt) {
    const int c = blockIdx.x;
    double* col = S + (size_t)c * nt;
    for (int r = (c / kPanelCols) * kPanelCols + static_cast<int>(threadIdx.x); r < nt; r += NT) col[r] = 0.0;
}

typedef double double4_t __attribute__((ext_vector_type(4)));
constexpr int KS = kSlab;

struct SlotLd {
    double a, b, d;
    bool ra, rb;
};
__device__ __forceinline__ SlotLd slot_ld(const SlotRec& m, const double* __restrict__ Lx,
                                          const double* __restrict__ dg, int lane) {
    const uint64_t below = (1ull << lane) - 1ull;
    SlotLd v;
    v.ra = (m.rmask >> lane) & 1ull;
    v.rb = (m.cmask >> lane) & 1ull;
    v.a = Lx[v.ra ? m.roff + __popcll(m.rmask & below) : m.roff];
    v.b = Lx[v.rb ? m.roff + m.cdelta + __popcll(m.cmask & below) : m.roff];
    v.d = dg[m.dk];
    return v;
}
__device__ __forceinline__ void slot_fin(const SlotLd& v, double& ra, double& rb) {
    ra = v.ra ? v.a : 0.0;
    rb = v.rb ? v.d * v.b : 0.0;
}

struct GatherTile {
    double* out;
    size_t ld;
    int nrow, ncol, row0, col0;
    double* dscale_col;
};

__device__ __forceinline__ GatherTile unit_tile(const PlanView& p, const TailView& tv, int u, int tail) {
    GatherTile g;
    if (tail < 0) {
        const int s = p.unit_sup[u], t = p.unit_tile[u];
        const int c0 = p.col0[s], nc = p.col0[s + 1] - c0;
        const int h = nc + (p.rowptr[s + 1] - p.rowptr[s]);
        const int rbase = t * TR;
        g.out = p.Lx + p.off[s] + rbase;
        g.ld = h;
        g.nrow = min(TR, h - rbase);
        g.ncol = nc;
        g.row0 = rbase;
        g.col0 = 0;
        g.dscale_col = t == 0 ? p.dscale + c0 : nullptr;
    } else {
        int bi = 0;
        while ((bi + 1) * (bi + 2) / 2 <= u) bi++;
        const int bj = u - bi * (bi + 1) / 2;
        g.out = tv.S + bi * TR + (size_t)(bj * TR) * tv.nt;
        g.ld = tv.nt;
        g.nrow = min(TR, tv.nt - bi * TR);
        g.ncol = min(TR, tv.nt - bj * TR);
        g.row0 = bi * TR;
        g.col0 = bj * TR;
        g.dscale_col = bi == bj ? p.dscale + tv.tc + bj * TR : nullptr;
    }
    return g;
}

__device__ void gather_acc(const PlanView& p, const SlotRec* __restrict__ recs, int kb, int ke, int dcol,
                           bool has_diag, double4_t (&acc)[2][2], double& dabs) {
    __shared__ double As[2][TR][KS + 1];
    __shared__ double Bs[2][TR][KS + 1];
    const int tid = threadIdx.x;
    const int wv = __builtin_amdgcn_readfirstlane(tid >> 6), lane = tid & 63;
    const int wr = (wv & 1) * 32, wc = (wv >> 1) * 32;
    const int li = lane & 15, lk = lane >> 4;
#pragma unroll
    for (int a = 0; a < 2; a++)
#pragma unroll
        for (int b = 0; b < 2; b++) acc[a][b] = (double4_t){0.0, 0.0, 0.0, 0.0};
    dabs = 0.0;
    const int nk = ke - kb, nslab = nk / KS;
    double ra[KS / 4], rb[KS / 4];
    const double* __restrict__ Lx = p.Lx;
    const double* __restrict__ dg = p.dg;
    const SlotRec* __restrict__ wrec = recs + kb + wv * (KS / 4);
    SlotRec mn[KS / 4];
    auto fetch = [&](int slab) {
#pragma unroll
        for (int j = 0; j < KS / 4; j++) mn[j] = wrec[slab * KS + j];
// ... 427 lines not shown
    for (int kk = 0; kk < PC; kk += 4) {
        double av[2], bv[2];
        for (int a = 0; a < 2; a++) av[a] = As[wr + a * 16 + li][kk + lk];
        for (int b = 0; b < 2; b++) bv[b] = Bs[wc + b * 16 + li][kk + lk];
        for (int a = 0; a < 2; a++)
            for (int b = 0; b < 2; b++) acc[a][b] = __builtin_amdgcn_mfma_f64_16x16x4f64(av[a], bv[b], acc[a][b], 0, 0, 0);
    }
    const bool diag_tile = bi == bj;
    double old[2][2][4];
#pragma unroll
    for (int a = 0; a < 2; a++)
#pragma unroll
        for (int b = 0; b < 2; b++)
#pragma unroll
            for (int i = 0; i < 4; i++) {
                const int rr = wr + a * 16 + (lane >> 4) + 4 * i;
                const int cc = wc + b * 16 + (lane & 15);
                const int rg = bi * TR + rr, cg = bj * TR + cc;
                const bool ok = rg < nt && cg < nt && !(diag_tile && cc > rr);
                old[a][b][i] = ok ? tv.S[rg + (size_t)cg * nt] : 0.0;
            }
#pragma unroll
    for (int a = 0; a < 2; a++)
#pragma unroll
        for (int b = 0; b < 2; b++)
#pragma unroll
            for (int i = 0; i < 4; i++) {
                const int rr = wr + a * 16 + (lane >> 4) + 4 * i;
                const int cc = wc + b * 16 + (lane & 15);
                const int rg = bi * TR + rr, cg = bj * TR + cc;
                if (rg >= nt || cg >= nt || (diag_tile && cc > rr)) continue;
                tv.S[rg + (size_t)cg * nt] = old[a][b][i] - acc[a][b][i];
            }
    if (diag_tile && tid < TR) {
        const int rg = bi * TR + tid;
        if (rg < nt) {
            double as = 0.0;
            for (int k = 0; k < nc; k++) as += fabs(As[tid][k] * Bs[tid][k]);
            p.dscale[tv.tc + rg] += as;
        }
    }
}

struct PermJobs {
    const double* fy[2];
    const double* fx[2];
    double* z[2];
    double* dy[2];
    double* dx[2];
    int mode[2];
};
__global__ void __launch_bounds__(NT)
k_perm_in2(int T, int m, const int* __restrict__ perm, PermJobs J, int* __restrict__ zi, double* __restrict__ zd) {
    const int v = blockIdx.x * NT + threadIdx.x, q = blockIdx.y;
    if (q == 0 && v < 2 && zi) { zi[v] = 0; zd[v] = 0.0; }
    if (v >= T) return;
    const int o = perm[v];
    J.z[q][v] = o < m ? J.fy[q][o] : J.fx[q][o - m];
}
__global__ void __launch_bounds__(NT)
k_perm_out2(int T, int m, const int* __restrict__ iperm, PermJobs J) {
    const int o = blockIdx.x * NT + threadIdx.x, q = blockIdx.y;
    if (o >= T) return;
    const double v = J.z[q][iperm[o]];
    double* dst = o < m ? J.dy[q] + o : J.dx[q] + (o - m);
    const int mode = J.mode[q];
    if (mode == 0) *dst = v;
    else if (mode == 1) *dst = *dst + v;
    else *dst = *dst - v;
}

__global__ void __launch_bounds__(NT)
k_perm_out(int T, int m, const int* __restrict__ iperm, const double* __restrict__ z, double* __restrict__ dy,
           double* __restrict__ dx, int mode) {
    const int o = blockIdx.x * NT + threadIdx.x;
    if (o >= T) return;
    const double v = z[iperm[o]];
    double* dst = o < m ? dy + o : dx + (o - m);
    if (mode == 0) *dst = v;
    else if (mode == 1) *dst = *dst + v;
    else *dst = *dst - v;
}

__device__ __forceinline__ void kkt_residual_body(
    int m, int n, const int* __restrict__ kAt, const int* __restrict__ iAt, const double* __restrict__ At,
    const int* __restrict__ kA, const int* __restrict__ iA, const double* __restrict__ A, const double* __restrict__ E,
    const double* __restrict__ D, const double* __restrict__ fy, const double* __restrict__ fx,
    const double* __restrict__ dy, const double* __restrict__ dx, double* __restrict__ ry, double* __restrict__ rx,
    double* __restrict__ part, int mrow, const double* __restrict__ axl, const int* __restrict__ kQ,
    const int* __restrict__ iQ, const double* __restrict__ Q, double qmax, int qthr,
    const double* __restrict__ qxl) {
    __shared__ double sh[kResThreads / 64];
    double mx = 0.0;
    for (int i = blockIdx.x * kResThreads + threadIdx.x; i < m + n; i += kRedBlocks * kResThreads) {
        if (i < m) {
            double s = 0.0;
            if (i >= mrow) s = axl[i - mrow];
            else
                s = sparse_dot(kAt[i], kAt[i + 1], At, iAt, dx);
            const double r = kQ ? fy[i] - ((s - E[i] * dy[i]) -
                                           qmax * (q_col_long(kQ, i, qthr) ? qxl[i]
                                                                           : sparse_dot(kQ[i], kQ[i + 1], Q, iQ, dy)))
                                : fy[i] - (s - E[i] * dy[i]);
            ry[i] = r;
            mx = fmax(mx, ref_abs(r));
        } else {
            const int j = i - m;
            double s = 0.0;
            s = sparse_dot(kA[j], kA[j + 1], A, iA, dy);
            const double r = fx[j] - (s + D[j] * dx[j]);
            rx[j] = r;
            mx = fmax(mx, ref_abs(r));
        }
    }
    mx = block_max_w<kResThreads / 64>(mx, sh);
    if (threadIdx.x == 0) part[blockIdx.x] = mx;
}


struct ResJobs {
    const double* fy[2];
    const double* fx[2];
    const double* dy[2];
    const double* dx[2];
    double* ry[2];
    double* rx[2];
    const double* axl[2];
    const double* qxl[2];
};
__global__ void __launch_bounds__(kResThreads)
k_kkt_residual2(int m, int n, const int* __restrict__ kAt, const int* __restrict__ iAt, const double* __restrict__ At,
                const int* __restrict__ kA, const int* __restrict__ iA, const double* __restrict__ A,
                const double* __restrict__ E, const double* __restrict__ D, ResJobs J, double* __restrict__ part,
                int mrow, const int* __restrict__ kQ, const int* __restrict__ iQ, const double* __restrict__ Q,
                double qmax, int qthr) {
    const int q = blockIdx.y;
    kkt_residual_body(m, n, kAt, iAt, At, kA, iA, A, E, D, J.fy[q], J.fx[q], J.dy[q], J.dx[q], J.ry[q], J.rx[q],
                      part + (size_t)q * kRedBlocks, mrow, J.axl[q], kQ, iQ, Q, qmax, qthr, J.qxl[q]);
}

__global__ void __launch_bounds__(NT)
k_min_abs_partial(const double* __restrict__ d, int T, double* __restrict__ part) {
    __shared__ double sh[4];
    double mn = HUGE_VAL;
    for (int i = blockIdx.x * NT + threadIdx.x; i < T; i += kRedBlocks * NT) mn = fmin(mn, ref_abs(d[i]));
    const double r = block_max(-mn, sh);
    if (threadIdx.x == 0) part[blockIdx.x] = r;
}

struct CopyOut {
    const double* src[4];
    double* dst[4];
    int m, n, R;
};
__global__ void __launch_bounds__(NT) k_copy_out(CopyOut c) {
    const int i = blockIdx.x * NT + threadIdx.x, per = c.m + c.n;
    if (i >= c.R * per) return;
    const int r = i / per, k = i - r * per;
    if (k < c.m) c.dst[2 * r][k] = c.src[2 * r][k];
    else c.dst[2 * r + 1][k - c.m] = c.src[2 * r + 1][k - c.m];
}
__global__ void k_pack_ints(const int* f, int n, double* out) {
    if (static_cast<int>(threadIdx.x) < n) reinterpret_cast<int*>(out)[threadIdx.x] = f[threadIdx.x];
}
__global__ void k_flag_to_scalar(const int* f, double* d) { d[0] = static_cast<double>(f[0]); }

}

KktDevice::KktDevice(int m, int n, const int* kA, const int* iA, const double* A, hipStream_t stream, int nforced,
                     const QBlock* qb)
    : m_(m), n_(n), T_(m + n), nforced_(nforced), stream_(stream) {
    if (qb && !qb->kQ) qb = nullptr;
    if (qb && nforced > 0) throw std::invalid_argument("kkt: a Q block with forced rows is not supported");
    QPattern qpat;
    if (qb) { qpat.kQ = qb->kQ; qpat.iQ = qb->iQ; }
    const auto st0 = std::chrono::steady_clock::now();
    auto mark = [&](const char* what) {
        if (knobs_.setup_times)
            std::fprintf(stderr, "setup %-28s %9.1f ms\n", what,
                         std::chrono::duration<double, std::milli>(std::chrono::steady_clock::now() - st0).count());
    };
    std::vector<int> kat, iat;
    std::vector<double> at;
    csc_transpose(m, n, kA, iA, A, kat, iat, at);
    const double tail_density = device_tail_density();
    mark("transpose");
    plan_ = build_kkt_plan(m, n, kA, iA, kat.data(), iat.data(), nforced, tail_density, qb ? &qpat : nullptr);
    mark("ordering + symbolic plan");
    h_.paths = kkt_paths(plan_, knobs_);
    int dev = 0, cus = 0;
    IPO_HIP_CHECK(hipGetDevice(&dev));
    IPO_HIP_CHECK(hipDeviceGetAttribute(&cus, hipDeviceAttributeMultiprocessorCount, dev));
    upload_plan(kA, iA, A, kat, iat, at, qb);
    mark("upload_plan");
    build_panel_units();
    mark("build_panel_units");
    {
        const SolveChunks ch = build_solve_chunks();
        mark("build_solve_chunks");
        const SweepOrder so = build_sweep_order(ch);
        mark("build_sweep_order");
        build_sync_free_plan(ch, so, cus);
        mark("build_sync_free_plan");
    }
    const VisitSlots vs = build_visit_slots(plan_, knobs_, h_.paths);
    mark("build_visit_slots");
    build_gather_chunks(vs);
    mark("build_gather_chunks");
    count_work();
    mark("count_work");
    build_slot_records(vs.kslot);
    mark("build_slot_records");
    setup_tail(cus);
    mark("setup_tail");
    alloc_numeric();
    mark("alloc_numeric");
}

void KktDevice::upload_plan(const int* kA, const int* iA, const double* A, const std::vector<int>& kat,
                            const std::vector<int>& iat, const std::vector<double>& at, const QBlock* qb) {
    const int m = m_, n = n_;
    if (nforced_ > 0) dLinkAx_.alloc(2 * static_cast<size_t>(nforced_));
    const int nz = kA[n];
    hipStream_t s = stream_;
    dkA_.upload(kA, n + 1, s);
    diA_.upload(iA, nz, s);
    dA_.upload(A, nz, s);
    dkAt_.upload(kat, s);
    diAt_.upload(iat, s);
    dAt_.upload(at, s);
// ... 112 lines not shown
    build(plan_.utasks, dusrc_);
    if (plan_.nt > 0) build(plan_.tail_tasks, dtsrc_);
    auto expand = [&](const std::vector<int>& kslot, const std::vector<TailTask>& ts, DevBuf<SlotRec>& dst) {
        const std::vector<SlotRec> v = ipo::build_slot_records(plan_, kslot, ts);
        dst.upload(v, s);
        IPO_HIP_CHECK(hipStreamSynchronize(s));
    };
    expand(h_.paths.visits ? kslot_v : plan_.kslot, plan_.utasks, dslot_rec_);
    if (plan_.nt > 0) expand(plan_.tail_kslot, plan_.tail_tasks, dtail_slot_rec_);
    dutasks_.upload(reinterpret_cast<const uint64_t*>(plan_.utasks.data()), plan_.utasks.size() * 4, s);
}

void KktDevice::setup_tail(int cus) {
    hipStream_t s = stream_;
    if (plan_.nt > 0) {
        dtail_task_ptr_.upload(plan_.tail_task_ptr, s);
        dtail_kslot_.upload(plan_.tail_kslot, s);
        dtail_kslot_ptr_.upload(plan_.tail_kslot_ptr, s);
        static_assert(sizeof(TailTask) == 32, "TailTask layout");
        dtail_tasks_.upload(reinterpret_cast<const uint64_t*>(plan_.tail_tasks.data()), plan_.tail_tasks.size() * 4, s);
        dW_.alloc(static_cast<size_t>(plan_.nt) * kPanelCols);
        dDepSt_.alloc(tail_dep_state_doubles(plan_.ntb));
        dDepI_.alloc(8);
        dChainGran_.alloc(ChainGran::words(plan_.ntb));
        dlead_ticket_.alloc(1);
        IPO_HIP_CHECK(hipMemsetAsync(dlead_ticket_.get(), 0, sizeof(int), s));
        lead_ticket_next_ = 0;
        IPO_HIP_CHECK(hipMemsetAsync(dChainGran_.get(), 0, dChainGran_.bytes(), s));
    }
    raise_sweep_lds(false);
    if (plan_.nt > 0 && plan_.ntb <= kTailSchedMaxBlocks) {
        TailSchedule ts = build_tail_schedule(plan_, knobs_, h_.paths, cus);
        if (knobs_.visit_sched) {
            dvisit_list_.upload(ts.visit_list, s);
            IPO_HIP_CHECK(hipStreamSynchronize(s));
            h_.visit_ptr = std::move(ts.visit_ptr);
        }
        if (h_.paths.tail_run) {
            static_assert(sizeof(SchedUint2) == sizeof(uint2), "SchedUint2 is uploaded as uint2");
            drun_items_.upload(reinterpret_cast<const uint2*>(ts.run_items.data()), ts.run_items.size(), s);
            h_.run_ptr = std::move(ts.run_ptr);
            drun_cnt_.alloc(RunCounters::words(plan_.ntb));
            if (h_.paths.run_winpub) {
                drun_pub_.alloc(2 * static_cast<size_t>(plan_.ntb) * 4 * kTailPubWin);
                drun_wflag_.alloc(static_cast<size_t>(plan_.ntb) * plan_.ntb * 4);
                IPO_HIP_CHECK(hipMemsetAsync(drun_wflag_.get(), 0, drun_wflag_.bytes(), s));
                run_epoch_ = 0;
            }
            IPO_HIP_CHECK(hipStreamSynchronize(s));
        }
    }
}

void KktDevice::alloc_numeric() {
    hipStream_t s = stream_;
    dLx_.alloc(plan_.lx_size > 0 ? plan_.lx_size : 1);
    dDg_.alloc(T_ > 0 ? T_ : 1);
    dLive_.alloc(T_ > 0 ? T_ : 1);
    dDscale_.alloc(T_ > 0 ? T_ : 1);
    dFlags_.alloc(kFlagWords);
    IPO_HIP_CHECK(hipMemsetAsync(dFlags_.get(), 0, dFlags_.bytes(), s));
    dSign_.upload(plan_.dsign, s);
    dZ_.alloc(2 * (T_ > 0 ? T_ : 1));
    dDy_.alloc(2 * (m_ > 0 ? m_ : 1));
    dRy_.alloc(2 * (m_ > 0 ? m_ : 1));
    dDx_.alloc(2 * (n_ > 0 ? n_ : 1));
    dRx_.alloc(2 * (n_ > 0 ? n_ : 1));
    dIncons_.alloc(2);
    dPart_.alloc(8 * kRedBlocks);
    dScal_.alloc(kScCount);
    dFacScal_.alloc(kFsCount);
    static_assert(kFlagReadWords * sizeof(int) <= (kFsCount - kFsFlags) * sizeof(double), "the packed flag words");
    dPrePart_.alloc(8 * kRedBlocks);
    IPO_HIP_CHECK(hipHostMalloc(reinterpret_cast<void**>(&hScal_), std::max(kScCount, kFsCount) * sizeof(double),
                                hipHostMallocDefault));
    IPO_HIP_CHECK(hipHostMalloc(reinterpret_cast<void**>(&hDepDone_), sizeof(int), hipHostMallocDefault));
    IPO_HIP_CHECK(hipEventCreate(&ev0_));
    IPO_HIP_CHECK(hipEventCreate(&ev1_));
    IPO_HIP_CHECK(hipEventCreate(&ev2_));
    IPO_HIP_CHECK(hipEventCreate(&ev3_));
    IPO_HIP_CHECK(hipEventCreateWithFlags(&ev_pre_fork_, hipEventDisableTiming));
    IPO_HIP_CHECK(hipEventCreateWithFlags(&ev_pre_done_, hipEventDisableTiming));
    IPO_HIP_CHECK(hipEventCreateWithFlags(&ev_run_reset_, hipEventDisableTiming));
    IPO_HIP_CHECK(hipStreamSynchronize(s));
}

void KktDevice::build_sync_free_plan(const SolveChunks& ch, const SweepOrder& so, int cus) {
    hipStream_t s = stream_;
    dyrow_ptr_.upload(plan_.yrow_ptr, s);
    const SyncFreePlan sf = ipo::build_sync_free_plan(plan_, knobs_, h_.paths, ch);
    const int ns = plan_.nsup;
    h_.sf_level = sf.sf_level;
    dyrow_idx_.upload(sf.yrow_idx, s);
    dybase_.upload(sf.ybase, s);
    if (sf.late_lists) {
        dylate_ptr_.upload(sf.ylate_ptr, s);
        dylate_idx_.upload(sf.ylate_idx.empty() ? std::vector<int>{0} : sf.ylate_idx, s);
        dpre_col_.upload(sf.pre_col.empty() ? std::vector<int>{0} : sf.pre_col, s);
        dpre_ptr_.upload(sf.pre_ptr, s);
        dpre_idx_.upload(sf.pre_idx.empty() ? std::vector<int>{0} : sf.pre_idx, s);
        IPO_HIP_CHECK(hipStreamSynchronize(s));
    }
    h_.ybuf_stride = sf.ybuf_stride;
    dYbuf_.alloc(2 * h_.ybuf_stride);
    h_.sweep = build_sweep_steps(plan_, knobs_, h_.paths, ch, so, sf, h_.paths.tail_blocked);
    if (sf.range(plan_)) {
        static_assert(sizeof(SchedInt2) == sizeof(int2), "SchedInt2 is uploaded as int2");
        dsf_items_f_.upload(reinterpret_cast<const int2*>(sf.items_f.data()), sf.items_f.size(), s);
#ifdef IPO_SF_STAMPS
        h_sf_items_f_ = sf.items_f;
#endif
        dsf_items_b_.upload(reinterpret_cast<const int2*>(sf.items_b.data()), sf.items_b.size(), s);
        dsf_need_.upload(sf.need, s);
        dsf_par_.upload(sf.par, s);
        dsf_zbase_.upload(sf.zbase, s);
        dsf_zpi_.upload(sf.zpi, s);
        h_.zpad_stride = sf.zpad_stride;
        dZpad_.alloc(2 * h_.zpad_stride);
        for (DevBuf<int>* b : {&dsf_fcnt_, &dsf_fflag_, &dsf_bcnt_, &dsf_bflag_}) {
            b->alloc(ns);
            IPO_HIP_CHECK(hipMemsetAsync(b->get(), 0, ns * sizeof(int), s));
        }
        dsf_ticket_.alloc(2);
        IPO_HIP_CHECK(hipMemsetAsync(dsf_ticket_.get(), 0, 2 * sizeof(int), s));
        sf_ticket_next_[0] = sf_ticket_next_[1] = 0;
        sf_grid_ = cus;
    }
    raise_sweep_lds(true);
    IPO_HIP_CHECK(hipStreamSynchronize(s));
}

KktDevice::~KktDevice() {
    dump_sf_stamps();
    if (knobs_.debug_redo)
        std::fprintf(stderr, "kkt: %ld factorisations, %ld redone; bails (unused) %ld, k_panel_w sparse %ld, tail %ld, "
                             "k_panel_s %ld; tail block columns repaired %ld in %ld rounds\n", tm_.factors,
                     tm_.panel_redos, tm_.redo_where[0], tm_.redo_where[1], tm_.redo_where[2], tm_.redo_where[3],
                     tm_.tail_repairs, tm_.tail_dep_rounds);
    if (knobs_.debug_redo) {
        std::fprintf(stderr, "kkt: forward pre-passes used %ld, discarded %ld\n", pre_used_, pre_discarded_);
        std::fprintf(stderr, "kkt: trailing leads used %ld, discarded %ld\n", lead_used_, lead_discarded_);
    }
    if (hScal_) (void)hipHostFree(hScal_);
    if (hDepDone_) (void)hipHostFree(hDepDone_);
    if (ev0_) (void)hipEventDestroy(ev0_);
    if (ev1_) (void)hipEventDestroy(ev1_);
    if (ev2_) (void)hipEventDestroy(ev2_);
    if (ev3_) (void)hipEventDestroy(ev3_);
    if (ev_pre_fork_) (void)hipEventDestroy(ev_pre_fork_);
    if (ev_pre_done_) (void)hipEventDestroy(ev_pre_done_);
    if (ev_run_reset_) (void)hipEventDestroy(ev_run_reset_);
    for (hipEvent_t e : kev_) (void)hipEventDestroy(e);
}

PlanView KktDevice::plan_view() const {
    PlanView v;
    v.col0 = dcol0_.get(); v.rowptr = drowptr_.get(); v.rows = drows_.get(); v.off = doff_.get();
    v.unit_sup = dunit_sup_.get(); v.unit_tile = dunit_tile_.get();
    v.task_ptr = dtask_ptr_.get(); v.task_pair = dtask_pair_.get();
    v.task_i0 = dtask_i0_.get(); v.task_i1 = dtask_i1_.get();
    v.upd_src = dupd_src_.get(); v.upd_r0 = dupd_r0_.get(); v.upd_r1 = dupd_r1_.get();
    v.relptr = drelptr_.get(); v.rel = drel_.get();
    v.Lx = dLx_.get(); v.dg = dDg_.get(); v.live = dLive_.get();
    v.flags = dFlags_.get();
    v.sign = dSign_.get();
    v.xcd = knobs_.update_xcd;
    v.dscale = dDscale_.get();
    v.tau = pivot_tol_;
    v.incons = dIncons_.get();
    v.ybase = dybase_.get();
    return v;
}

TailView KktDevice::tail_view() const {
    TailView t;
    t.S = dLx_.get() + plan_.off_tail;
    t.nt = plan_.nt;
    t.ntb = plan_.ntb;
    t.tc = plan_.tail_c0;
    t.task_ptr = dtail_task_ptr_.get();
    t.tasks = reinterpret_cast<const TailTask*>(dtail_tasks_.get());
    t.W = dW_.get();
    t.vk = knobs_.visit_blocks;
    if (!h_.visit_ptr.empty()) {
        t.vlist = dvisit_list_.get();
        t.vptr = h_.visit_ptr.data();
    }
    t.dep = tail_repair() ? knobs_.tail_spec : 0;
    t.sdep = knobs_.sparse_dep;
    return t;
}

void KktDevice::dump_factor(const double* dE, const double* dD, double eps_in) {
    if (knobs_.dump_dir.empty()) return;
    std::vector<double> E(m_), D(n_), dg(T_), dsc(T_);
    std::vector<int> live(T_);
    IPO_HIP_CHECK(hipStreamSynchronize(stream_));
    if (m_) IPO_HIP_CHECK(hipMemcpy(E.data(), dE, m_ * sizeof(double), hipMemcpyDeviceToHost));
    if (n_) IPO_HIP_CHECK(hipMemcpy(D.data(), dD, n_ * sizeof(double), hipMemcpyDeviceToHost));
    dLive_.download(live.data(), T_, stream_);
    dDg_.download(dg.data(), T_, stream_);
    dDscale_.download(dsc.data(), T_, stream_);
    IPO_HIP_CHECK(hipStreamSynchronize(stream_));
    char path[4096];
    std::snprintf(path, sizeof path, "%s/f%04d.bin", knobs_.dump_dir.c_str(), dump_count_++);
    FILE* f = std::fopen(path, "wb");
    if (!f) return;
    const int hdr[4] = {m_, n_, T_, ndep_};
    const double eps[2] = {eps_in, epsdiag_};
    std::fwrite(hdr, sizeof(int), 4, f);
    std::fwrite(eps, sizeof(double), 2, f);
    std::fwrite(E.data(), sizeof(double), m_, f);
    std::fwrite(D.data(), sizeof(double), n_, f);
    std::fwrite(plan_.perm.data(), sizeof(int), T_, f);
    std::fwrite(live.data(), sizeof(int), T_, f);
    std::fwrite(dg.data(), sizeof(double), T_, f);
    std::fwrite(dsc.data(), sizeof(double), T_, f);
    std::fclose(f);
}

void KktDevice::factor(const double* dE, const double* dD, const PrePass* pre) {
    const double eps_in = epsdiag_;
    drop_prepass();
    try {
        factor_core(dE, dD, pre);
    } catch (...) {
        if (pre_state_ != kPreNone) (void)hipStreamWaitEvent(stream_, ev_pre_done_, 0);
        drop_prepass();
        throw;
    }
    dump_factor(dE, dD, eps_in);
}

void KktDevice::factor_core(const double* dE, const double* dD, const PrePass* pre) {
    const bool repair = tail_repair();
    const bool ok = factor_pass(dE, dD, use_panel_, use_panel_, pre);
    if (!ok) {
        tm_.panel_redos++;
        for (int b = 0; b < 4; b++) tm_.redo_where[b] += (verdict_.bail >> b) & 1;
        if (repair && verdict_.tail_only()) repair_tail();
        else if (!factor_pass(dE, dD, false, repair) && repair && verdict_.tail_only()) repair_tail();
    }
    tm_.factors++;
    if (timing_)
        for (int ph : {kPhGather, kPhDiag, kPhTrsm, kPhSyrk, kPhTail}) tm_.phase_count[ph]++;
    ndep_ = verdict_.ndep_all;
    if (pre_state_ == kPreEnqueued) {
        if (ok && ndep_ == 0) pre_state_ = kPreValid;
        else drop_prepass();
    }
    if (verdict_.min_d < 1.0e-14) epsdiag_ *= 10;
    if (knobs_.epsdiag_max > 0.0 && epsdiag_ > knobs_.epsdiag_max) epsdiag_ = knobs_.epsdiag_max;
}

bool KktDevice::factor_pass(const double* dE, const double* dD, bool fused, bool tail_fused, const PrePass* pre) {
    hipStream_t s = stream_;
    if (timing_) IPO_HIP_CHECK(hipEventRecord(ev0_, s));
    const PlanView pv = plan_view();
    const int nz = static_cast<int>(plan_.amap.size());
    if (plan_.nt > 0 && !xch_) {
        if (plan_.off_tail > 0) IPO_HIP_CHECK(hipMemsetAsync(dLx_.get(), 0, plan_.off_tail * sizeof(double), s));
        hipLaunchKernelGGL(k_zero_tail_lower, dim3(plan_.nt), dim3(NT), 0, s, dLx_.get() + plan_.off_tail, plan_.nt);
    } else {
        IPO_HIP_CHECK(hipMemsetAsync(dLx_.get(), 0, dLx_.bytes(), s));
    }
    if (nz > 0) hipLaunchKernelGGL(k_assemble_A, dim3(ceil_div(nz, NT)), dim3(NT), 0, s, nz, dA_.get(), damap_.get(), dLx_.get());
    if (qnz_ > 0)
        hipLaunchKernelGGL(k_assemble_Q, dim3(ceil_div(qnz_, NT)), dim3(NT), 0, s, qnz_, dQ_.get(), dqmap_.get(),
                           static_cast<double>(qmax_), dLx_.get());
    hipLaunchKernelGGL(k_assemble_diag, dim3(ceil_div(T_, NT)), dim3(NT), 0, s, T_, m_, dperm_.get(), dE, dD, epsdiag_,
                       ddslot_.get(), dLx_.get(), dLive_.get(), dDscale_.get(), shard_minor() ? plan_.tail_c0 : T_,
                       dFlags_.get(), dkQ_.get() ? dQdiag_.get() : static_cast<const double*>(nullptr),
                       static_cast<double>(qmax_));
    const TailView tv = tail_view();
    if (!prepass_eligible(pre, fused, tail_fused)) pre = nullptr;
    enqueue_levels(pv, tv, fused, s, pre);
    if (plan_.nt > 0) {
        xsum(tv.S, static_cast<size_t>(plan_.nt) * plan_.nt, RedOp::Sum);
        xsum(dDscale_.get() + plan_.tail_c0, plan_.nt, RedOp::Sum);
        if (tail_fused && h_.paths.tail_run) {
            launch_tail_from(0, true);
        } else if (tail_fused) {
            ph_begin(s);
            for (int t = 0; t < plan_.ntb; t++) launch_tail_step(pv, tv, t, s);
            ph_end(kPhTail, plan_.ntb, s);
        } else
        for (int kb = 0; kb < plan_.ntb; kb++) {
            const int k0 = kb * kPanelCols, nc = std::min(kPanelCols, plan_.nt - k0);
            const int below = plan_.nt - k0 - nc;
            ph_begin(s);
            {
                launch_diag(pv, nullptr, 0, 1, tv, kb, s);
                ph_end(kPhDiag, 1, s);
                if (below > 0) {
                    ph_begin(s);
                    launch_trsm(pv, 0, -1, tv, kb, s);
                    ph_end(kPhTrsm, 1, s);
                }
            }
            if (below > 0) {
                const int nb = plan_.ntb - kb - 1;
                ph_begin(s);
                hipLaunchKernelGGL(k_tail_syrk, dim3(nb * (nb + 1) / 2), dim3(NT), 0, s, pv, tv, kb);
                ph_end(kPhSyrk, 1, s);
            }
        }
    }
    if (pre) IPO_HIP_CHECK(hipStreamWaitEvent(s, ev_pre_done_, 0));
    return finish_pass(fused || tail_fused);
}

bool KktDevice::prepass_eligible(const PrePass* pre, bool fused, bool tail_fused) const {
    return knobs_.prepass && pre && (pre->R == 1 || pre->R == 2) && pre->stream && pre->stream != stream_ &&
           pre->ready && fused && tail_fused && h_.paths.tail_run && h_.sweep.split > 0 && !xch_ && !timing_;
}

void KktDevice::enqueue_pass_head(int R, double* const* dfy, double* const* dfx, double* part, hipStream_t s) {
    RedJobs j{};
    j.nj = 2 * R;
    PermJobs J{};
    for (int r = 0; r < R; r++) {
        j.a[2 * r] = dfx[r]; j.b[2 * r] = nullptr; j.len[2 * r] = n_; j.op[2 * r] = 1;
        j.a[2 * r + 1] = dfy[r]; j.b[2 * r + 1] = nullptr; j.len[2 * r + 1] = m_; j.op[2 * r + 1] = 1;
        J.fy[r] = dfy[r];
        J.fx[r] = dfx[r];
        J.z[r] = dZ_.get() + static_cast<size_t>(r) * T_;
    }
    launch_reduce(j, part, dScal_.get() + kScMaxbc, s);
    xsum(dScal_.get() + kScMaxbc, 2 * R, RedOp::Max);
    hipLaunchKernelGGL(k_perm_in2, dim3(ceil_div(T_, NT), R), dim3(NT), 0, s, T_, m_, dperm_.get(), J, dIncons_.get(),
                       sweep_eps());
}

void KktDevice::enqueue_prepass(const PrePass& pre) {
    hipStream_t q = pre.stream;
    IPO_HIP_CHECK(hipEventRecord(ev_pre_fork_, stream_));
    IPO_HIP_CHECK(hipStreamWaitEvent(q, ev_pre_fork_, 0));
    IPO_HIP_CHECK(hipStreamWaitEvent(q, pre.ready, 0));
    enqueue_pass_head(pre.R, pre.dfy, pre.dfx, dPrePart_.get(), q);
    run_prepass_steps(pre.R, q);
    IPO_HIP_CHECK(hipEventRecord(ev_pre_done_, q));
    pre_req_ = pre;
    pre_state_ = kPreEnqueued;
    pre_lead_ = false;
    lead_pending_ = h_.sweep.lead_end > 0 ? knobs_.lead_trail_mode(plan_.ntb) : 0;
}

void KktDevice::enqueue_levels(const PlanView& pv, const TailView& tv, bool fused, hipStream_t s, const PrePass* pre) {
    for (int l = 0; l < plan_.nlevels; l++) {
        const int u0 = plan_.unit_level_ptr[l], u1 = plan_.unit_level_ptr[l + 1];
        if (u1 <= u0) continue;
        if (l > 0) {
            ph_begin(s);
            const int nl = launch_gather(pv, tv, -1, l, s);
            ph_end(kPhGather, nl, s);
        }
        const int q0 = plan_.level_ptr[l], q1 = plan_.level_ptr[l + 1];
        ph_begin(s);
        if (fused && h_.split_level[l]) {
            launch_diag(pv, dlevel_sups_.get(), q0, q1 - q0, tv, 0, s);
            launch_trsm(pv, u0, u1 - u0, tv, 0, s);
            ph_end(kPhDiag, 2, s);
        } else if (fused) {
            const int nsm = h_.small_ptr[l + 1] - h_.small_ptr[l], nfu = h_.fu_ptr[l + 1] - h_.fu_ptr[l];
            const int n1 = h_.small1_cnt[l];
            if (knobs_.merge_levels && nfu > 0 && nsm > n1) {
                launch_panel_small(pv, dsmall_sups_.get(), h_.small_ptr[l], n1, tv.sdep, s, n1);
                launch_panel_ws(pv, dfu_sup_.get(), dfu_j_.get(), h_.fu_ptr[l], nfu, tv, dsmall_sups_.get(),
                                h_.small_ptr[l] + n1, nsm - n1, tv.sdep, s);
                ph_end(kPhDiag, 1 + (n1 > 0), s);
            } else {
                launch_panel_small(pv, dsmall_sups_.get(), h_.small_ptr[l], nsm, tv.sdep, s, n1);
                launch_panel(pv, dfu_sup_.get(), dfu_j_.get(), h_.fu_ptr[l], nfu, tv, -1, s);
                ph_end(kPhDiag, (nsm > 0) + (nfu > 0), s);
            }
        } else {
            launch_diag(pv, dlevel_sups_.get(), q0, q1 - q0, tv, 0, s);
            ph_end(kPhDiag, 1, s);
            ph_begin(s);
            launch_trsm(pv, u0, u1 - u0, tv, 0, s);
            ph_end(kPhTrsm, 1, s);
        }
    }
    if (pre) enqueue_prepass(*pre);
    if (plan_.nt > 0) {
        ph_begin(s);
        const int nl = launch_gather(pv, tv, 0, plan_.nlevels, s);
        ph_end(kPhGather, nl, s);
    }
}

bool KktDevice::finish_pass(bool fused) {
    hipStream_t s = stream_;
    IPO_HIP_CHECK(hipGetLastError());
    hipLaunchKernelGGL(k_min_abs_partial, dim3(kRedBlocks), dim3(NT), 0, s, dDg_.get(), T_, dPart_.get());
    if (xch_) {
        static_assert(kFsNegMinD == 0 && kFsNdepMax == 1 && kFsBailMax == 2, "one allreduce over the three");
        hipLaunchKernelGGL(k_finish_reduce, dim3(1), dim3(kRedThreads), 0, s, dPart_.get(), 1, 1u,
                           dFacScal_.get() + kFsNegMinD);
        hipLaunchKernelGGL(k_flag_to_scalar, dim3(1), dim3(1), 0, s, dFlags_.get() + kFlagNdep,
                           dFacScal_.get() + kFsNdepMax);
        hipLaunchKernelGGL(k_flag_to_scalar, dim3(1), dim3(1), 0, s, dFlags_.get() + kFlagBail,
                           dFacScal_.get() + kFsBailMax);
        xsum(dFacScal_.get(), kFsFlags, RedOp::Max);
        hipLaunchKernelGGL(k_pack_ints, dim3(1), dim3(kFlagReadWords), 0, s, dFlags_.get(), kFlagReadWords,
                           dFacScal_.get() + kFsFlags);
    } else {
        hipLaunchKernelGGL(k_finish_reduce_pack, dim3(1), dim3(kRedThreads), 0, s, dPart_.get(), 1, 1u,
                           dFacScal_.get() + kFsNegMinD, static_cast<const int*>(dFlags_.get()), kFlagReadWords,
                           dFacScal_.get() + kFsFlags);
    }
    IPO_HIP_CHECK(hipMemcpyAsync(hScal_, dFacScal_.get(), kFsCount * sizeof(double), hipMemcpyDeviceToHost, s));
    if (timing_) IPO_HIP_CHECK(hipEventRecord(ev1_, s));
    IPO_HIP_CHECK(hipStreamSynchronize(s));
    if (gst_n_ > 0) {
        std::vector<long long> st(1024 * 8);
        IPO_HIP_CHECK(hipMemcpy(st.data(), dGStamp_.get(), st.size() * sizeof(long long), hipMemcpyDeviceToHost));
        long long t0 = st[0];
        for (int b = 0; b < std::min(gst_n_, 1024); b++) t0 = std::min(t0, st[b * 8]);
        std::fprintf(stderr, "gather stamps group %d, %d workgroups (us from first start: start rec val mfma acc put slots)\n",
                     gst_group_, gst_n_);
        for (int b = 0; b < std::min(gst_n_, 1024); b++) {
            const long long* q = st.data() + b * 8;
            std::fprintf(stderr, "  wg %4d: %6.2f %6.2f %6.2f %6.2f %6.2f %6.2f  %lld\n", b, (q[0] - t0) / 100.0,
                         (q[1] - t0) / 100.0, (q[2] - t0) / 100.0, (q[3] - t0) / 100.0, (q[4] - t0) / 100.0,
                         (q[5] - t0) / 100.0, q[6]);
        }
        gst_n_ = 0;
        gst_group_ = -1;
    }
    {
        int f[kFlagReadWords];
        std::memcpy(f, hScal_ + kFsFlags, sizeof(f));
        FactorVerdict& v = verdict_;
        v.min_d = -hScal_[kFsNegMinD];
        v.ndep = f[kFlagNdep];
        v.bail = f[kFlagBail];
        v.tail_block = f[kFlagTailBlock];
        v.ndep_all = xch_ ? static_cast<int>(hScal_[kFsNdepMax]) : v.ndep;
        v.bail_all = xch_ ? static_cast<int>(hScal_[kFsBailMax]) : v.bail;
    }
    if (timing_) {
        float ms = 0;
        IPO_HIP_CHECK(hipEventElapsedTime(&ms, ev0_, ev1_));
        tm_.factor_ms += ms;
        ph_collect();
    }
    return !(fused && verdict_.any_bail());
}

void KktDevice::launch_tail_from(int t0, bool reset) {
    hipStream_t s = stream_;
    const PlanView pv = plan_view();
    const RunCounters cnt = run_counters();
    const size_t ncnt = reset ? RunCounters::words(plan_.ntb) : 1;
    IPO_HIP_CHECK(hipMemsetAsync(cnt.ticket, 0, ncnt * sizeof(int), s));
    TailRun rc;
    rc.items = drun_items_.get() + h_.run_ptr[t0];
    rc.n = h_.run_ptr[plan_.ntb] - h_.run_ptr[t0];
    rc.t0 = t0;
    rc.ticket = cnt.ticket;
    rc.pdone = cnt.pdone;
    rc.vseq = cnt.vseq;
    rc.cdone = cnt.cdone;
    if (h_.paths.run_winpub) {
        if (run_epoch_ == INT_MAX) {
            IPO_HIP_CHECK(hipMemsetAsync(drun_wflag_.get(), 0, drun_wflag_.bytes(), s));
            run_epoch_ = 0;
        }
        rc.pub = drun_pub_.get();
        rc.wflag = drun_wflag_.get();
        rc.pread = cnt.pread;
        if (!reset) IPO_HIP_CHECK(hipMemsetAsync(rc.pread + t0, 0, (plan_.ntb - t0) * sizeof(int), s));
        rc.epoch = ++run_epoch_;
    }
    if (lead_pending_ == 2) IPO_HIP_CHECK(hipEventRecord(ev_run_reset_, s));
    ph_begin(s);
    launch_tail_run(pv, tail_view(), rc, s);
    ph_end(kPhTail, rc.n > 0, s);
// ... 58 lines not shown
        if (!dGStamp_.get()) dGStamp_.alloc(1024 * 8);
        stq = dGStamp_.get();
        gst_n_ = c1 - c0;
    }
    if (h_.ck_kind[group] == 2) {
        hipLaunchKernelGGL(k_update_quad, dim3(c1 - c0), dim3(NT), 0, s, pv, tv, recs, dck_u_.get(), dck_b_.get(),
                           dck_e_.get(), dck_part_.get(), c0, stq);
        return 1;
    }
    if (h_.ck_kind[group] == 1) {
        if (h_.ck_wide[group])
        hipLaunchKernelGGL(k_update_flat<4>, dim3(c1 - c0), dim3(NT), 0, s, pv, tv, tail, recs, dck_u_.get(),
                           dck_b_.get(), dck_e_.get(), dck_part_.get(), c0, dPartialTile_.get(), dck_q_.get(),
                           dsp_p0_.get(), dsp_n_.get(), dSplitCnt_.get(), stq);
        else
        hipLaunchKernelGGL(k_update_flat<1>, dim3(c1 - c0), dim3(NT), 0, s, pv, tv, tail, recs, dck_u_.get(),
                           dck_b_.get(), dck_e_.get(), dck_part_.get(), c0, dPartialTile_.get(), dck_q_.get(),
                           dsp_p0_.get(), dsp_n_.get(), dSplitCnt_.get(), stq);
        return 1;
    }
    const int occ = knobs_.update_occ;
    auto go = [&](auto kern) {
        hipLaunchKernelGGL(kern, dim3(c1 - c0), dim3(NT), 0, s, pv, tv, tail, recs, dck_u_.get(), dck_b_.get(),
                           dck_e_.get(), dck_part_.get(), c0, dPartialTile_.get(), dck_q_.get(), dsp_p0_.get(),
                           dsp_n_.get(), dSplitCnt_.get());
    };
    if (h_.ck_wide[group]) {
        go(k_update<4, 1>);
    } else {
        if (occ == 4) go(k_update<1, 4>);
        else go(k_update<1, 1>);
    }
    return 1;
}

hipEvent_t KktDevice::next_event() {
    if (kev_used_ == kev_.size()) {
        hipEvent_t e;
        IPO_HIP_CHECK(hipEventCreate(&e));
        kev_.push_back(e);
    }
    return kev_[kev_used_++];
}

void KktDevice::ph_begin(hipStream_t s) {
    if (!timing_) return;
    mark_b_ = next_event();
    IPO_HIP_CHECK(hipEventRecord(mark_b_, s));
}

void KktDevice::ph_end(int phase, int launches, hipStream_t s) {
    if (!timing_) return;
    hipEvent_t e = next_event();
    IPO_HIP_CHECK(hipEventRecord(e, s));
    marks_.push_back({mark_b_, e, phase, launches});
}

void KktDevice::ph_collect() {
    for (const PhaseMark& mk : marks_) {
        float ms = 0;
        IPO_HIP_CHECK(hipEventElapsedTime(&ms, mk.b, mk.e));
        tm_.phase_ms[mk.phase] += ms;
        tm_.phase_launches[mk.phase] += mk.launches;
    }
    marks_.clear();
    kev_used_ = 0;
}

void KktDevice::launch_q_long(const double* v, double* out) {
    ipo::launch_q_long(q_long_n_, dQLongCols_.get(), dkQ_.get(), diQ_.get(), dQ_.get(), v, out, stream_);
}

void KktDevice::set_long_rows(int row0) {
    if (xch_ || row0 < 0 || row0 >= m_) return;
    long_row0_ = row0;
    dLongAx_.alloc(2 * static_cast<size_t>(m_ - row0));
}

void KktDevice::solve_multi(int R, const double* dE, const double* dD, double* const* dfy, double* const* dfx,
                            int* ok) {
    hipStream_t s = stream_;
    if (timing_) IPO_HIP_CHECK(hipEventRecord(ev0_, s));
    const int m = m_, n = n_, T = T_;
    const bool pre_lead = pre_lead_;
    const bool pre = take_prepass(R, dfy, dfx);
    if (!pre && R > 0) enqueue_pass_head(R, dfy, dfx, dPart_.get(), s);
    double maxbc[2] = {0.0, 0.0}, rs[2] = {HUGE_VAL, HUGE_VAL}, rs_old[2] = {HUGE_VAL, HUGE_VAL};
    int pass[2] = {0, 0};
    bool active[2] = {R > 0, R > 1};
    auto zv = [&](int r) { return dZ_.get() + (size_t)r * T; };
    auto dyv = [&](int r) { return dDy_.get() + (size_t)r * m; };
    auto dxv = [&](int r) { return dDx_.get() + (size_t)r * n; };
    auto ryv = [&](int r) { return dRy_.get() + (size_t)r * m; };
    auto rxv = [&](int r) { return dRx_.get() + (size_t)r * n; };
    int incons[2] = {0, 0};
    while (active[0] || active[1]) {
        const bool first = pass[0] + pass[1] == 0;
        if (!first) {
            PermJobs J{};
            int na = 0;
            for (int r = 0; r < R; r++)
                if (active[r]) {
                    J.fy[na] = ryv(r);
                    J.fx[na] = rxv(r);
                    J.z[na] = zv(r);
                    na++;
                }
            hipLaunchKernelGGL(k_perm_in2, dim3(ceil_div(T, NT), na), dim3(NT), 0, s, T, m, dperm_.get(), J,
                               dIncons_.get(), sweep_eps());
        }
        eps_cleared_ = true;
        const size_t fwd_first = first && pre ? static_cast<size_t>(pre_lead ? h_.sweep.lead_end : h_.sweep.split) : 0;
        if (active[0] && active[1]) rawsolve(zv(0), 2, fwd_first);
        else rawsolve(zv(active[0] ? 0 : 1), 1, fwd_first);
        eps_cleared_ = false;
        int nq = 0;
        {
            PermJobs P{};
            ResJobs J{};
            const int mrow = xch_ ? m - nforced_ : long_row0_ >= 0 ? long_row0_ : m;
            for (int r = 0; r < R; r++) {
                if (!active[r]) continue;
                P.z[nq] = zv(r); P.dy[nq] = dyv(r); P.dx[nq] = dxv(r); P.mode[nq] = pass[r] == 0 ? 0 : 1;
                J.fy[nq] = dfy[r]; J.fx[nq] = dfx[r]; J.dy[nq] = dyv(r); J.dx[nq] = dxv(r);
                J.ry[nq] = ryv(r); J.rx[nq] = rxv(r);
                J.axl[nq] = xch_ ? dLinkAx_.get() + (size_t)r * nforced_
                                 : long_row0_ >= 0 ? dLongAx_.get() + (size_t)r * (m - long_row0_) : nullptr;
                J.qxl[nq] = q_long_n_ > 0 ? dLongQ_.get() + (size_t)r * m : nullptr;
                nq++;
            }
            hipLaunchKernelGGL(k_perm_out2, dim3(ceil_div(T, NT), nq), dim3(NT), 0, s, T, m, diperm_.get(), P);
            for (int q = 0; q < nq; q++) {
                double* axl = const_cast<double*>(J.axl[q]);
                if (xch_) {
                    launch_link_ax(mrow, m, dkAt_.get(), diAt_.get(), dAt_.get(), J.dx[q], axl, s);
                    xsum(axl, nforced_, RedOp::Sum);
                } else if (long_row0_ >= 0) {
                    launch_link_ax(mrow, m, dkAt_.get(), diAt_.get(), dAt_.get(), J.dx[q], axl, s);
                }
                if (q_long_n_ > 0) launch_q_long(J.dy[q], const_cast<double*>(J.qxl[q]));
            }
            hipLaunchKernelGGL(k_kkt_residual2, dim3(kRedBlocks, nq), dim3(kResThreads), 0, s, m, n, dkAt_.get(),
                               diAt_.get(), dAt_.get(), dkA_.get(), diA_.get(), dA_.get(), dE, dD, J, dPart_.get(), mrow,
                               dkQ_.get() ? dkQ_.get() : static_cast<const int*>(nullptr), diQ_.get(), dQ_.get(),
                               static_cast<double>(qmax_), q_long_min());
        }
        if (xch_) {
            hipLaunchKernelGGL(k_finish_reduce, dim3(1), dim3(kRedThreads), 0, s, dPart_.get(), nq, (1u << nq) - 1u,
                               dScal_.get() + kScRes);
            xsum(dScal_.get() + kScRes, nq, RedOp::Max);
            hipLaunchKernelGGL(k_pack_ints, dim3(1), dim3(2), 0, s, dIncons_.get(), 2, dScal_.get() + kScIncons);
        } else {
            hipLaunchKernelGGL(k_finish_reduce_pack, dim3(1), dim3(kRedThreads), 0, s, dPart_.get(), nq,
                               (1u << nq) - 1u, dScal_.get() + kScRes, static_cast<const int*>(dIncons_.get()), 2,
                               dScal_.get() + kScIncons);
        }
        IPO_HIP_CHECK(hipMemcpyAsync(hScal_, dScal_.get(), (first ? kScMaxbc + 2 * R : kScReadLater) * sizeof(double),
                                     hipMemcpyDeviceToHost, s));
        IPO_HIP_CHECK(hipStreamSynchronize(s));
        if (first)
            for (int r = 0; r < R; r++) {
                const double* mb = hScal_ + kScMaxbc + 2 * r;
                maxbc[r] = (mb[0] > mb[1] ? mb[0] : mb[1]) + 1;
            }
        int slot_incons[2];
        std::memcpy(slot_incons, hScal_ + kScIncons, sizeof(slot_incons));
        const double* res = hScal_ + kScRes;
        int q = 0;
        for (int r = 0; r < R; r++) {
            if (!active[r]) continue;
            incons[r] = slot_incons[q];
            rs_old[r] = rs[r];
            rs[r] = res[q++];
            pass[r]++;
            active[r] = rs[r] > 1.0e-10 * maxbc[r] && rs[r] < rs_old[r] / 2;
        }
    }
    CopyOut co{};
    for (int r = 0; r < R; r++) {
        if (rs[r] > rs_old[r] && pass[r] > 1)
            hipLaunchKernelGGL(k_perm_out, dim3(ceil_div(T, NT)), dim3(NT), 0, s, T, m, diperm_.get(), zv(r), dyv(r),
                               dxv(r), 2);
        co.src[2 * r] = dyv(r); co.dst[2 * r] = dfy[r];
        co.src[2 * r + 1] = dxv(r); co.dst[2 * r + 1] = dfx[r];
    }
    co.m = m;
    co.n = n;
    co.R = R;
    if (R > 0 && m + n > 0) hipLaunchKernelGGL(k_copy_out, dim3(ceil_div(R * (m + n), NT)), dim3(NT), 0, s, co);
    if (timing_) {
        IPO_HIP_CHECK(hipEventRecord(ev1_, s));
        IPO_HIP_CHECK(hipStreamSynchronize(s));
        float ms = 0;
        IPO_HIP_CHECK(hipEventElapsedTime(&ms, ev0_, ev1_));
        tm_.solve_ms += ms;
    }
    tm_.solves += R;
    last_passes_ = pass[0] + pass[1];
    for (int r = 0; r < R; r++) ok[r] = incons[r] ? 0 : 1;
}

bool KktDevice::take_prepass(int R, double* const* dfy, double* const* dfx) {
    bool same = pre_state_ == kPreValid && !timing_ && pre_req_.R == R;
    for (int r = 0; same && r < R; r++) same = pre_req_.dfy[r] == dfy[r] && pre_req_.dfx[r] == dfx[r];
    if (!same) {
        drop_prepass();
        return false;
    }
    pre_state_ = kPreNone;
    pre_used_++;
    if (pre_lead_) lead_used_++;
    pre_lead_ = false;
    return true;
}

int KktDevice::solve(const double* dE, const double* dD, double* dfy, double* dfx) {
    int ok[1];
    solve_multi(1, dE, dD, &dfy, &dfx, ok);
    return ok[0];
}

int KktDevice::solve2(const double* dE, const double* dD, double* dfy1, double* dfx1, double* dfy2, double* dfx2) {
    double* fy[2] = {dfy1, dfy2};
    double* fx[2] = {dfx1, dfx2};
    int ok[2];
    solve_multi(2, dE, dD, fy, fx, ok);
    return ok[0] && ok[1];
}

void KktDevice::download_factor(double* lx, double* d, int* live) const {
    if (lx) dLx_.download(lx, plan_.lx_size, stream_);
    if (d) dDg_.download(d, T_, stream_);
    if (live) dLive_.download(live, T_, stream_);
    IPO_HIP_CHECK(hipStreamSynchronize(stream_));
}

}
```

### linear-programming-vanderbei_amd/csrc/kkt_kernels.h

```cpp
#pragma once
#include <hip/hip_runtime.h>

#include <cstdint>
#include <vector>

#include "kkt_device.h"
#include "kkt_plan.h"

namespace ipo {

constexpr int TR = kTileRows;
constexpr int PC = kPanelCols;
constexpr int NT = 256;

struct PlanView {
    const int* col0;
    const int* rowptr;
    const int* rows;
    const int64_t* off;
    const int* unit_sup;
    const int* unit_tile;
    const int* task_ptr;
    const int* task_pair;
    const int* task_i0;
    const int* task_i1;
    const int* upd_src;
    const int* upd_r0;
    const int* upd_r1;
    const int64_t* relptr;
    const int* rel;
    double* Lx;
    double* dg;
    int* live;
    int* flags;
    const int* sign;
    double* dscale;
    double tau;
    int* incons;
    const int* ybase;
    int xcd;
};

static __device__ __forceinline__ int xcd_chunk(int b, int G) {
    const int q = G >> 3, r = G & 7, x = b & 7, i = b >> 3;
    return (x < r ? x * (q + 1) : r * (q + 1) + (x - r) * q) + i;
}

static __device__ __forceinline__ void sc1_store(double* p, double v) {
    __hip_atomic_store(p, v, __ATOMIC_RELAXED, __HIP_MEMORY_SCOPE_AGENT);
}
static __device__ __forceinline__ double sc1_load(const double* p) {
    return __hip_atomic_load(const_cast<double*>(p), __ATOMIC_RELAXED, __HIP_MEMORY_SCOPE_AGENT);
}
static __device__ __forceinline__ int sc1_load_int(const int* p) {
    return __hip_atomic_load(const_cast<int*>(p), __ATOMIC_RELAXED, __HIP_MEMORY_SCOPE_AGENT);
}
template <bool SC>
static __device__ __forceinline__ double ld_h(const double* p) {
    if constexpr (SC) return sc1_load(p);
    else return *p;
}
template <bool SC>
static __device__ __forceinline__ void st_h(double* p, double v) {
    if constexpr (SC) sc1_store(p, v);
    else *p = v;
}

typedef double double2_t __attribute__((ext_vector_type(2)));
static __device__ __forceinline__ __amdgpu_buffer_rsrc_t buf_rsrc(const double* base) {
    return __builtin_amdgcn_make_buffer_rsrc(const_cast<double*>(base), 0, 0x7fffffff, 0x00020000);
}
template <bool SC>
static __device__ __forceinline__ double2_t ld2_h(__amdgpu_buffer_rsrc_t rs, int voff, int soff) {
    return __builtin_bit_cast(double2_t, __builtin_amdgcn_raw_buffer_load_b128(rs, voff, soff, SC ? 16 : 0));
}
template <bool SC>
static __device__ __forceinline__ void st2_h(__amdgpu_buffer_rsrc_t rs, int voff, int soff, double2_t v) {
    typedef unsigned int u32x4 __attribute__((ext_vector_type(4)));
    __builtin_amdgcn_raw_buffer_store_b128(__builtin_bit_cast(u32x4, v), rs, voff, soff, SC ? 16 : 0);
}

static __device__ __forceinline__ double lane_bcast(double v, int j) {
    const long long b = __double_as_longlong(v);
    const int lo = __builtin_amdgcn_readlane(static_cast<int>(b), j);
    const int hi = __builtin_amdgcn_readlane(static_cast<int>(b >> 32), j);
    return __longlong_as_double((static_cast<long long>(hi) << 32) | static_cast<unsigned int>(lo));
}

void launch_diag(const PlanView& pv, const int* level_sups, int q0, int count, const TailView& tv, int kb,
                 hipStream_t s);
void launch_trsm(const PlanView& pv, int u0, int count, const TailView& tv, int kb, hipStream_t s);
void launch_panel(const PlanView& pv, const int* fu_sup, const int* fu_j, int f0, int count, const TailView& tv,
                  int kb, hipStream_t s);
void launch_tail_step(const PlanView& pv, const TailView& tv, int t, hipStream_t s);
void launch_tail_run(const PlanView& pv, const TailView& tv, const TailRun& rc, hipStream_t s);
void launch_tail_dep_round(const PlanView& pv, const TailView& tv, int kb, int round, double* st, int* sti,
                           hipStream_t s);
size_t tail_dep_state_doubles(int ntb);
void launch_tail_colupdate(const PlanView& pv, const TailView& tv, int t, hipStream_t s);
void launch_tail_restore(const PlanView& pv, const TailView& tv, int kb, hipStream_t s);
void launch_panel_ws(const PlanView& pv, const int* fu_sup, const int* fu_j, int f0, int nfu, const TailView& tv,
                     const int* ssups, int s0, int nsm, int dep, hipStream_t s);
void launch_panel_small(const PlanView& pv, const int* sups, int q0, int count, int dep, hipStream_t s, int n1 = 0);

}
```

### linear-programming-vanderbei_amd/csrc/kkt_knobs.h

```cpp
#pragma once
#include <algorithm>
#include <cstdlib>
#include <string>

#include "kkt_plan.h"

namespace ipo {

constexpr int kTailVisitBlocks = 4;
constexpr int kTailVisitLatest = 4;
constexpr int kLongQCol = 256;
constexpr int kTrailHelpers = 8;
constexpr int kTrailMinBlocks = 4;

struct KktKnobs {

    bool panel = true;
    bool merge_levels = true;
    bool sf = true;
    bool overlap = true;
    bool prepass = true;
    int lead_trail = -1;
    int lead_trail_mode(int ntb) const { return lead_trail >= 0 ? lead_trail : ntb >= kTrailMinBlocks ? 2 : 0; }
    int lead_helpers = kTrailHelpers;
    bool chain_lead = true;
    bool chain_pairs = false;
    bool tail_run = true;
    bool tail_winpub = true;
    bool visit_sched = true;
    bool visit_xcd = true;
    bool tail_repair = true;
    int tail_spec = 1;
    int sparse_dep = 1;
    int visits = -1;
    int gather_flat = 1;
    bool gather_quad = true;
    int small_leaves = -1;
    int panel_split = 768;
    int ax_blocks = 1;
    int ax_jds = -1;


    int visit_blocks = kTailVisitBlocks;
    int visit_latest = kTailVisitLatest;
    int visit_slabs = kVisitSlots / kSlab;
    int min_chunk = 64;
    int sf_width = -1;
    int update_xcd = 1024;
    int update_occ = 4;
    int dot_segmin = -1;
    int q_long = kLongQCol;


    bool setup_times = false;
    bool debug_redo = false;
    bool trace_full = false;
    std::string dump_dir;
    int gather_stamps = -1;
    double epsdiag_max = 0.0;
    double pivtol = 1.0e-17;
    std::string sf_stamps_file;

    bool deep_tree(int nlevels) const { return visits < 0 ? nlevels >= kVisitLevels : visits != 0; }

    static KktKnobs from_env() {
        const auto flag = [](const char* name, bool dflt) {
            const char* e = std::getenv(name);
            return e ? std::atoi(e) != 0 : dflt;
        };
        const auto num = [](const char* name, int dflt) {
            const char* e = std::getenv(name);
            return e ? std::atoi(e) : dflt;
        };
        const auto real = [](const char* name, double dflt) {
            const char* e = std::getenv(name);
            return e ? std::atof(e) : dflt;
        };
        const auto text = [](const char* name) {
            const char* e = std::getenv(name);
            return std::string(e ? e : "");
        };
        const auto set = [](const char* name) { return std::getenv(name) != nullptr; };
        KktKnobs k;
        k.panel = flag("IPO_HIP_PANEL", true);
        k.merge_levels = flag("IPO_HIP_MERGE_LEVELS", true);
        k.sf = flag("IPO_HIP_SF", true);
        k.overlap = flag("IPO_HIP_OVERLAP", true);
        k.prepass = flag("IPO_HIP_PREPASS", true);
        k.lead_trail = num("IPO_HIP_LEAD_TRAIL", -1);
        if (k.lead_trail < 0 || k.lead_trail > 2) k.lead_trail = -1;
        k.lead_helpers = std::max(1, num("IPO_HIP_LEAD_HELPERS", kTrailHelpers));
        k.chain_lead = flag("IPO_HIP_CHAIN_LEAD", true);
        k.chain_pairs = flag("IPO_HIP_CHAIN_PAIRS", false);
        k.tail_run = flag("IPO_HIP_TAIL_RUN", true);
        k.tail_winpub = flag("IPO_HIP_TAIL_WINPUB", true);
        k.visit_sched = flag("IPO_HIP_VISIT_SCHED", true);
        k.visit_xcd = flag("IPO_HIP_VISIT_XCD", true);
        k.tail_repair = flag("IPO_HIP_TAIL_REPAIR", true);
        k.tail_spec = num("IPO_HIP_TAIL_SPEC", 1);
        k.sparse_dep = num("IPO_HIP_SPARSE_DEP", 1);
        if (set("IPO_HIP_VISITS")) k.visits = flag("IPO_HIP_VISITS", false);
        k.gather_flat = num("IPO_HIP_GATHER_FLAT", 1);
        k.gather_quad = flag("IPO_HIP_GATHER_QUAD", true);
        if (set("IPO_HIP_SMALL_LEAVES")) k.small_leaves = std::max(0, num("IPO_HIP_SMALL_LEAVES", 0));
        k.panel_split = std::max(0, num("IPO_HIP_PANEL_SPLIT", 768));
        k.ax_blocks = std::max(1, num("IPO_HIP_AX_BLOCKS", 1));
        if (set("IPO_HIP_AX_JDS")) k.ax_jds = flag("IPO_HIP_AX_JDS", false);
        k.visit_blocks = std::max(1, num("IPO_HIP_VISIT_BLOCKS", kTailVisitBlocks));
        k.visit_latest = std::max(1, num("IPO_HIP_VISIT_LATEST", kTailVisitLatest));
        if (set("IPO_HIP_VISIT_SLOTS")) k.visit_slabs = std::max(1, num("IPO_HIP_VISIT_SLOTS", 0) / kSlab);
        if (set("IPO_HIP_MIN_CHUNK")) k.min_chunk = std::max(kSlab, num("IPO_HIP_MIN_CHUNK", 0) / kSlab * kSlab);
        if (set("IPO_HIP_SF_WIDTH")) k.sf_width = std::max(1, num("IPO_HIP_SF_WIDTH", 0));
        k.update_xcd = std::max(0, num("IPO_HIP_UPDATE_XCD", 1024));
        k.update_occ = num("IPO_HIP_UPDATE_OCC", 4);
        if (set("IPO_HIP_DOT_SEGMIN")) k.dot_segmin = std::max(0, num("IPO_HIP_DOT_SEGMIN", 0));
        k.q_long = std::max(0, num("IPO_HIP_Q_LONG", kLongQCol));
        k.setup_times = set("IPO_HIP_SETUP_TIMES");
        k.debug_redo = set("IPO_HIP_DEBUG_REDO");
        k.trace_full = set("IPO_HIP_TRACE_FULL");
        k.dump_dir = text("IPO_HIP_DUMP_DIR");
        k.gather_stamps = num("IPO_HIP_GATHER_STAMPS", -1);
        k.epsdiag_max = real("IPO_HIP_EPSDIAG_MAX", 0.0);
        k.pivtol = real("IPO_HIP_PIVTOL", 1.0e-17);
        k.sf_stamps_file = text("IPO_SF_STAMPS_FILE");
        return k;
    }
};

}
```

### linear-programming-vanderbei_amd/csrc/kkt_sweep.hip

```cpp
#include <hip/hip_runtime.h>

#include <algorithm>
#include <array>
#include <climits>
#include <cstdio>
#include <initializer_list>
#include <map>
#include <stdexcept>
#include <string>
#include <vector>

#include "dev_common.h"
#include "kkt_device.h"
#include "kkt_kernels.h"

namespace ipo {

namespace {

__device__ __forceinline__ int opaque_lane() {
    int lane = threadIdx.x & 63;
    asm volatile("" : "+v"(lane));
    return lane;
}
// ... 2115 lines not shown
        case kSwTailChain:
            if (forward)
                hipLaunchKernelGGL(k_tail_fwd_chain<R>, dim3(plan_.ntb), dim3(NT), kChainLds, s, pv, tv, V, epsp,
                                   dChainGran_.get(), ++chain_epoch_);
            else
                hipLaunchKernelGGL(k_tail_bwd_chain<R>, dim3(plan_.ntb), dim3(NT), kChainLds, s, pv, tv, V, epsp,
                                   dChainGran_.get(), ++chain_epoch_);
            break;
        case kSwTailPair:
            hipLaunchKernelGGL(k_tail_bwd_pair<R>, dim3((plan_.ntb + 1) / 2), dim3(NT), kPairBwdLds, s, pv, tv, V, epsp,
                               dChainGran_.get(), ++chain_epoch_);
            break;
        case kSwTailBlock: {
            const int kb = step.a;
            if (forward) {
                const int below = nt - std::min(nt, (kb + 1) * kPanelCols);
                hipLaunchKernelGGL(k_tail_fwd, dim3(std::max(1, ceil_div(below, 64))), dim3(NT), 0, s, pv, tv, kb, dz,
                                   epsp);
            } else {
                const int left = kb * kPanelCols;
                hipLaunchKernelGGL(k_tail_bwd, dim3(std::max(1, ceil_div(left, 64))), dim3(NT), 0, s, pv, tv, kb, dz,
                                   epsp);
            }
            break;
        }
        case kSwTailDscale:
            hipLaunchKernelGGL(k_tail_dscale, dim3(ceil_div(nt, NT)), dim3(NT), 0, s, pv, tv, dz, epsp);
            break;
        default:
            throw std::logic_error("sweep: unknown step kind");
        }
        launched++;
    }
    return launched;
}

void KktDevice::run_prepass_steps(int R, hipStream_t q) {
    double* epsp = sweep_eps();
    const size_t split = static_cast<size_t>(h_.sweep.split);
    if (R == 2) run_sweep_steps<2>(h_.sweep.fwd, true, dZ_.get(), epsp, 0, split, q);
    else run_sweep_steps<1>(h_.sweep.fwd, true, dZ_.get(), epsp, 0, split, q);
}

void KktDevice::launch_lead_trail(int R, hipStream_t s, bool beside) {
    const PlanView pv = plan_view();
    const TailView tv = tail_view();
    const SweepVecs V{dZ_.get(), static_cast<size_t>(T_), dYbuf_.get(), h_.ybuf_stride};
    const int nhb = std::max(0, plan_.ntb - 1 - kLeadBlocks);
    const int grid = 1 + (beside ? std::min(nhb, knobs_.lead_helpers) : nhb);
    const double* epsp = sweep_eps();
    gran_t* gran = dChainGran_.get();
    gran_t* pgran = gran + ChainGran::part_at(plan_.ntb);
    const RunCounters cnt = run_counters();
    if (R == 2)
        hipLaunchKernelGGL((k_tail_fwd_lead<2, true>), dim3(grid), dim3(kLeadNT), kLeadTrailLds, s, pv, tv, V, epsp, gran,
                           pgran, ++chain_epoch_, cnt.lead_ticket, 0, static_cast<const int*>(cnt.cdone));
    else
        hipLaunchKernelGGL((k_tail_fwd_lead<1, true>), dim3(grid), dim3(kLeadNT), kLeadTrailLds, s, pv, tv, V, epsp, gran,
                           pgran, ++chain_epoch_, cnt.lead_ticket, 0, static_cast<const int*>(cnt.cdone));
}

int KktDevice::sf_tbase(int d, int nitems, hipStream_t s) {
    const long long draw = static_cast<long long>(nitems) + std::min(sf_grid_, nitems);
    if (sf_ticket_next_[d] + draw > (1LL << 30)) {
        IPO_HIP_CHECK(hipMemsetAsync(dsf_ticket_.get() + d, 0, sizeof(int), s));
        sf_ticket_next_[d] = 0;
    }
    const int base = static_cast<int>(sf_ticket_next_[d]);
    sf_ticket_next_[d] += draw;
    return base;
}

void KktDevice::tail_rhs_begin(double* dz, int R) {
    if (!shard_minor()) return;
    for (int r = 0; r < R; r++)
        IPO_HIP_CHECK(hipMemsetAsync(dz + (size_t)r * T_ + plan_.tail_c0, 0, sizeof(double) * plan_.nt, stream_));
}
void KktDevice::tail_rhs_end(double* dz, int R) {
    for (int r = 0; r < R; r++) xsum(dz + (size_t)r * T_ + plan_.tail_c0, plan_.nt, RedOp::Sum);
}

void KktDevice::rawsolve(double* dz, int R, size_t fwd_first) {
    hipStream_t s = stream_;
    double* epsp = sweep_eps();
    if (ndep_ > 0) {
        RedJobs j{};
        j.nj = R;
        for (int r = 0; r < R; r++) { j.a[r] = dz + (size_t)r * T_; j.b[r] = nullptr; j.len[r] = n_; j.op[r] = 1; }
        launch_reduce(j, dPart_.get(), epsp, s);
        hipLaunchKernelGGL(k_scale_scalar, dim3(1), dim3(64), 0, s, epsp, R, 1.0e-6);
        xsum(epsp, R, RedOp::Max);
    } else if (!eps_cleared_) {
        IPO_HIP_CHECK(hipMemsetAsync(epsp, 0, R * sizeof(double), s));
    }
    if (R == 2 && !h_.paths.tail_blocked) {
        sweep<2>(dz, epsp, fwd_first);
    } else {
        for (int r = 0; r < R; r++) sweep<1>(dz + (size_t)r * T_, epsp + r, fwd_first);
    }
    tm_.rawsolves += R;
}

}
```

Measured before the change: 317.8 iterations/s.

## Fuse IPM glue kernels with last-block-arrives epilogues and pre-assemble next factor

Folds the small single-thread glue kernels (dphi, finish reduce, theta) into the preceding reduction kernels. A last-arriving-workgroup counter lets the final block compute the scalar epilogue, and the same pattern is applied to the factor min-diag and residual reductions. It also precomputes the next iteration's scaling and matrix assembly and clears factor storage early on a side stream. The aim is fewer tiny launches and serialization bubbles per iteration, at the cost of atomic counters, cross-block memory-ordering subtleties, and more complex state tracking between factor and solve.

```diff
diff --git a/linear-programming-vanderbei_amd/csrc/dev_common.h b/linear-programming-vanderbei_amd/csrc/dev_common.h
--- a/linear-programming-vanderbei_amd/csrc/dev_common.h
+++ b/linear-programming-vanderbei_amd/csrc/dev_common.h
@@ -12,6 +12,34 @@
 
 __device__ __forceinline__ double ref_max(double x, double y) { return x > y ? x : y; }
 __device__ __forceinline__ double ref_abs(double x) { return x > 0 ? x : -x; }
+
+static __device__ __forceinline__ void sc1_store(double* p, double v) {
+    __hip_atomic_store(p, v, __ATOMIC_RELAXED, __HIP_MEMORY_SCOPE_AGENT);
+}
+static __device__ __forceinline__ double sc1_load(const double* p) {
+    return __hip_atomic_load(const_cast<double*>(p), __ATOMIC_RELAXED, __HIP_MEMORY_SCOPE_AGENT);
+}
+static __device__ __forceinline__ int sc1_load_int(const int* p) {
+    return __hip_atomic_load(const_cast<int*>(p), __ATOMIC_RELAXED, __HIP_MEMORY_SCOPE_AGENT);
+}
+
+__device__ __forceinline__ bool arrive_last(int* cnt, int n, int* sh_last) {
+    asm volatile("s_waitcnt vmcnt(0)" ::: "memory");
+    __syncthreads();
+    if (threadIdx.x == 0) {
+        const int prev = __hip_atomic_fetch_add(cnt, 1, __ATOMIC_RELAXED, __HIP_MEMORY_SCOPE_AGENT);
+        if (prev == n - 1) __hip_atomic_store(cnt, 0, __ATOMIC_RELAXED, __HIP_MEMORY_SCOPE_AGENT);
+        *sh_last = prev == n - 1;
+    }
+    __syncthreads();
+    return *sh_last != 0;
+}
+__device__ __forceinline__ bool arrive_last_lane(int* cnt, int n) {
+    asm volatile("s_waitcnt vmcnt(0)" ::: "memory");
+    const int prev = __hip_atomic_fetch_add(cnt, 1, __ATOMIC_RELAXED, __HIP_MEMORY_SCOPE_AGENT);
+    if (prev == n - 1) __hip_atomic_store(cnt, 0, __ATOMIC_RELAXED, __HIP_MEMORY_SCOPE_AGENT);
+    return prev == n - 1;
+}
 
 template <int N>
 __device__ __forceinline__ double dpp_row_down(double v) {
@@ -123,6 +151,22 @@
     if (threadIdx.x == 0) r = fmax(fmax(sh[0], sh[1]), fmax(sh[2], sh[3]));
     __syncthreads();
     return r;
+}
+
+struct PackFinish {
+    int* cnt = nullptr;
+    double* out = nullptr;
+    const int* f = nullptr;
+    int nf = 0;
+    double* outi = nullptr;
+};
+__device__ __forceinline__ void finish_max_pack(const double* part, int nq, const PackFinish& fin, double* sh) {
+    for (int q = 0; q < nq; q++) {
+        const double v = threadIdx.x < kRedBlocks ? sc1_load(part + q * kRedBlocks + threadIdx.x) : 0.0;
+        const double r = block_max(v, sh);
+        if (threadIdx.x == 0) fin.out[q] = r;
+    }
+    if (static_cast<int>(threadIdx.x) < fin.nf) reinterpret_cast<int*>(fin.outi)[threadIdx.x] = fin.f[threadIdx.x];
 }
 
 __global__ void __launch_bounds__(kRedThreads)
@@ -151,6 +195,20 @@
 }
 extern bool g_ordered_reductions;
 void launch_reduce(const RedJobs& jobs, double* part, double* out, hipStream_t st);
+
+__device__ __forceinline__ void hsd_dphi_body(const double* red, double* dst, double gamma, double delta, double mu,
+                                              double phi, double psi) {
+    const double dphi = (red[0] - red[1] + gamma) / (red[2] - red[3] - psi / phi);
+    const double dpsi = delta * mu / phi - psi - (psi / phi) * dphi;
+    dst[0] = dphi;
+    dst[1] = dpsi;
+}
+struct DphiEpilogue {
+    int* cnt = nullptr;
+    double* dst = nullptr;
+    double gamma = 0.0, delta = 0.0, mu = 0.0, phi = 0.0, psi = 0.0;
+};
+bool launch_reduce_dphi(const RedJobs& jobs, double* out, const DphiEpilogue& epi, hipStream_t st);
 double dot_ordered_host(const double* a, const double* b, int n);
 
 void launch_link_ax(int mrow, int m, const int* kAt, const int* iAt, const double* At, const double* x, double* out,
diff --git a/linear-programming-vanderbei_amd/csrc/dev_common.hip b/linear-programming-vanderbei_amd/csrc/dev_common.hip
--- a/linear-programming-vanderbei_amd/csrc/dev_common.hip
+++ b/linear-programming-vanderbei_amd/csrc/dev_common.hip
@@ -53,8 +53,21 @@
 
 constexpr int kOrdThreads = 256;
 
+__device__ __forceinline__ void ordered_put(double* out, int j, double v, const DphiEpilogue& epi) {
+    if (!epi.cnt) {
+        out[j] = v;
+        return;
+    }
+    sc1_store(out + j, v);
+    if (!arrive_last_lane(epi.cnt, static_cast<int>(gridDim.x))) return;
+    double red[4];
+#pragma unroll
+    for (int k = 0; k < 4; k++) red[k] = sc1_load(out + k);
+    hsd_dphi_body(red, epi.dst, epi.gamma, epi.delta, epi.mu, epi.phi, epi.psi);
+}
+
 __global__ void __launch_bounds__(kOrdThreads)
-k_reduce_ordered(RedJobs jobs, double* __restrict__ out) {
+k_reduce_ordered(RedJobs jobs, double* out, DphiEpilogue epi) {
     const int j = blockIdx.x;
     const double* a = jobs.a[j];
     const double* b = jobs.b[j];
@@ -81,7 +94,7 @@
             }
         }
         acc = block_max(acc, sh);
-        if (tid == 0) out[j] = acc;
+        if (tid == 0) ordered_put(out, j, acc, epi);
         return;
     }
     constexpr int CH = 4096;
@@ -149,7 +162,7 @@
         for (; i < nz; i++) s += comp[buf][i];
         __hip_atomic_store(&freed[buf], k + 1, __ATOMIC_RELEASE, __HIP_MEMORY_SCOPE_WORKGROUP);
     }
-    out[j] = s;
+    ordered_put(out, j, s, epi);
 }
 
 double dot_ordered_host(const double* a, const double* b, int n) {
@@ -422,7 +435,7 @@
 
 void launch_reduce(const RedJobs& jobs, double* part, double* out, hipStream_t st) {
     if (g_ordered_reductions) {
-        hipLaunchKernelGGL(k_reduce_ordered, dim3(jobs.nj), dim3(kOrdThreads), 0, st, jobs, out);
+        hipLaunchKernelGGL(k_reduce_ordered, dim3(jobs.nj), dim3(kOrdThreads), 0, st, jobs, out, DphiEpilogue{});
         bool longdot = false;
         for (int j = 0; j < jobs.nj; j++) longdot |= job_segmented(jobs, j);
         if (longdot) {
@@ -439,4 +452,13 @@
     IPO_HIP_CHECK(hipGetLastError());
 }
 
-}
+bool launch_reduce_dphi(const RedJobs& jobs, double* out, const DphiEpilogue& epi, hipStream_t st) {
+    if (!g_ordered_reductions || jobs.nj != 4 || !epi.cnt) return false;
+    for (int j = 0; j < jobs.nj; j++)
+        if (job_segmented(jobs, j)) return false;
+    hipLaunchKernelGGL(k_reduce_ordered, dim3(jobs.nj), dim3(kOrdThreads), 0, st, jobs, out, epi);
+    IPO_HIP_CHECK(hipGetLastError());
+    return true;
+}
+
+}
diff --git a/linear-programming-vanderbei_amd/csrc/ipm.h b/linear-programming-vanderbei_amd/csrc/ipm.h
--- a/linear-programming-vanderbei_amd/csrc/ipm.h
+++ b/linear-programming-vanderbei_amd/csrc/ipm.h
@@ -99,6 +99,7 @@
     DevBuf<double> b_, c_, x_, y_, w_, z_;
     DevBuf<double> rho_, sig_, D_, E_, fx_, fy_, gx_, gy_, dx_, dy_, dz_, dw_;
     DevBuf<double> part_, part2_, scal_, lax_;
+    DevBuf<int> glue_cnt_;
     hipStream_t side_ = nullptr;
     hipEvent_t ev_step_ = nullptr, ev_side_ = nullptr;
     double* hs_ = nullptr;
diff --git a/linear-programming-vanderbei_amd/csrc/ipm_device.hip b/linear-programming-vanderbei_amd/csrc/ipm_device.hip
--- a/linear-programming-vanderbei_amd/csrc/ipm_device.hip
+++ b/linear-programming-vanderbei_amd/csrc/ipm_device.hip
@@ -66,14 +66,13 @@
     if (threadIdx.x == 0) { part[blockIdx.x] = sr; part[kRedBlocks + blockIdx.x] = ss; }
 }
 
-__global__ void __launch_bounds__(NT)
-k_hsd_directions(int m, int n, const double* __restrict__ dphip, double delta, double mu, const double* __restrict__ fx,
-                 const double* __restrict__ gx, const double* __restrict__ fy, const double* __restrict__ gy,
-                 const double* __restrict__ x, const double* __restrict__ z, const double* __restrict__ y,
-                 const double* __restrict__ w, const double* __restrict__ D, const double* __restrict__ E,
-                 double* __restrict__ dx, double* __restrict__ dz, double* __restrict__ dy, double* __restrict__ dw,
-                 double* __restrict__ part) {
-    __shared__ double sh[4];
+__device__ __forceinline__ double
+hsd_directions_body(int m, int n, const double* __restrict__ dphip, double delta, double mu, const double* __restrict__ fx,
+                    const double* __restrict__ gx, const double* __restrict__ fy, const double* __restrict__ gy,
+                    const double* __restrict__ x, const double* __restrict__ z, const double* __restrict__ y,
+                    const double* __restrict__ w, const double* __restrict__ D, const double* __restrict__ E,
+                    double* __restrict__ dx, double* __restrict__ dz, double* __restrict__ dy, double* __restrict__ dw,
+                    double* sh) {
     const double dphi = *dphip;
     double th = 0.0;
     for (int i = blockIdx.x * NT + threadIdx.x; i < m + n; i += kRedBlocks * NT) {
@@ -92,7 +91,18 @@
             th = fmax(th, -ddw / w[j]);
         }
     }
-    th = block_max(th, sh);
+    return block_max(th, sh);
+}
+
+__global__ void __launch_bounds__(NT)
+k_hsd_directions(int m, int n, const double* __restrict__ dphip, double delta, double mu, const double* __restrict__ fx,
+                 const double* __restrict__ gx, const double* __restrict__ fy, const double* __restrict__ gy,
+                 const double* __restrict__ x, const double* __restrict__ z, const double* __restrict__ y,
+                 const double* __restrict__ w, const double* __restrict__ D, const double* __restrict__ E,
+                 double* __restrict__ dx, double* __restrict__ dz, double* __restrict__ dy, double* __restrict__ dw,
+                 double* __restrict__ part) {
+    __shared__ double sh[4];
+    const double th = hsd_directions_body(m, n, dphip, delta, mu, fx, gx, fy, gy, x, z, y, w, D, E, dx, dz, dy, dw, sh);
     if (threadIdx.x == 0) part[blockIdx.x] = th;
 }
 
@@ -121,14 +131,10 @@
 }
 
 __global__ void k_hsd_dphi(double* sc, double gamma, double delta, double mu, double phi, double psi) {
-    const double* red = sc + kIsRed;
-    const double dphi = (red[0] - red[1] + gamma) / (red[2] - red[3] - psi / phi);
-    const double dpsi = delta * mu / phi - psi - (psi / phi) * dphi;
-    sc[kIsDphi] = dphi;
-    sc[kIsDphi + 1] = dpsi;
-}
-
-__global__ void k_hsd_theta(double* sc, double phi, double psi) {
+    hsd_dphi_body(sc + kIsRed, sc + kIsDphi, gamma, delta, mu, phi, psi);
+}
+
+__device__ __forceinline__ void hsd_theta_body(double* sc, double phi, double psi) {
     const double dphi = sc[kIsDphi], dpsi = sc[kIsDphi + 1];
     double theta = sc[kIsRed];
     if (theta < -dphi / phi) theta = -dphi / phi;
@@ -137,6 +143,36 @@
     sc[kIsTheta] = theta;
     sc[kIsPhiNext] = phi + theta * dphi;
     sc[kIsPhiNext + 1] = psi + theta * dpsi;
+}
+__global__ void k_hsd_theta(double* sc, double phi, double psi) { hsd_theta_body(sc, phi, psi); }
+
+__global__ void __launch_bounds__(NT)
+k_hsd_directions_theta(int m, int n, double delta, double mu, const double* __restrict__ fx,
+                       const double* __restrict__ gx, const double* __restrict__ fy, const double* __restrict__ gy,
+                       const double* __restrict__ x, const double* __restrict__ z, const double* __restrict__ y,
+                       const double* __restrict__ w, const double* __restrict__ D, const double* __restrict__ E,
+                       double* __restrict__ dx, double* __restrict__ dz, double* __restrict__ dy,
+                       double* __restrict__ dw, double* part, double* sc, double phi, double psi, int* cnt) {
+    static_assert(kRedBlocks == NT, "the last workgroup's thread t takes partial t, as k_finish_reduce does");
+    __shared__ double sh[4];
+    __shared__ int last;
+    const double th = hsd_directions_body(m, n, sc + kIsDphi, delta, mu, fx, gx, fy, gy, x, z, y, w, D, E, dx, dz, dy,
+                                          dw, sh);
+    if (threadIdx.x == 0) sc1_store(part + blockIdx.x, th);
+    if (!arrive_last(cnt, kRedBlocks, &last)) return;
+    const double r = block_max(sc1_load(part + threadIdx.x), sh);
+    if (threadIdx.x == 0) {
+        sc[kIsRed] = r;
+        hsd_theta_body(sc, phi, psi);
+    }
+}
+
+DphiEpilogue dphi_epilogue(int* cnt, double* sc, double gamma, double delta, double mu, double phi, double psi) {
+    DphiEpilogue e;
+    e.cnt = cnt;
+    e.dst = sc + kIsDphi;
+    e.gamma = gamma; e.delta = delta; e.mu = mu; e.phi = phi; e.psi = psi;
+    return e;
 }
 
 __global__ void __launch_bounds__(NT)
@@ -511,6 +547,8 @@
     part_.alloc(8 * kRedBlocks);
     part2_.alloc(8 * kRedBlocks);
     scal_.alloc(kIsCount);
+    glue_cnt_.alloc(2);
+    IPO_HIP_CHECK(hipMemsetAsync(glue_cnt_.get(), 0, glue_cnt_.bytes(), stream_));
     IPO_HIP_CHECK(hipStreamCreateWithFlags(&side_, hipStreamNonBlocking));
     IPO_HIP_CHECK(hipEventCreateWithFlags(&ev_step_, hipEventDisableTiming));
     IPO_HIP_CHECK(hipEventCreateWithFlags(&ev_side_, hipEventDisableTiming));
@@ -607,6 +645,9 @@
         std::fflush(tr);
     }
     KktDevice& K = *kkt_;
+    const bool glue = overlap && knobs_.glue;
+    const bool glue_asm = glue && !opt.timing && K.can_step_assemble();
+    bool assembled = false;
     int status = 5, iter;
     for (iter = 0; iter < opt.max_iter; iter++) {
         RedJobs j{};
@@ -634,8 +675,9 @@
                                scal_.get() + kIsNorm2);
             IPO_HIP_CHECK(hipMemcpyAsync(hs_, scal_.get(), kIsCount * sizeof(double), hipMemcpyDeviceToHost, side_));
             IPO_HIP_CHECK(hipEventRecord(ev_side_, side_));
-            hipLaunchKernelGGL(k_hsd_scaling, dim3(gv), dim3(NT), 0, s, m, n, x_.get(), y_.get(), w_.get(), z_.get(),
-                               E_.get(), D_.get());
+            if (!assembled)
+                hipLaunchKernelGGL(k_hsd_scaling, dim3(gv), dim3(NT), 0, s, m, n, x_.get(), y_.get(), w_.get(), z_.get(),
+                                   E_.get(), D_.get());
             spec = K.host_state();
             KktDevice::PrePass pre;
             pre.R = 2;
@@ -644,10 +686,11 @@
             pre.stream = side_;
             pre.ready = ev_side_;
             try {
-                K.factor(E_.get(), D_.get(), &pre);
+                K.factor(E_.get(), D_.get(), &pre, assembled);
             } catch (...) {
                 spec_err = std::current_exception();
             }
+            assembled = false;
             IPO_HIP_CHECK(hipEventSynchronize(ev_side_));
         } else {
             launch_reduce(j, part_.get(), scal_.get(), s);
@@ -704,6 +747,7 @@
         }
         K.solve2(E_.get(), D_.get(), fy_.get(), fx_.get(), gy_.get(), gx_.get());
         res->refine_passes += K.last_passes();
+        const bool fuse_next = glue_asm && iter + 1 < opt.max_iter;
 
         RedJobs q{};
         q.nj = 4;
@@ -712,17 +756,37 @@
         q.a[1] = b_.get(); q.b[1] = fy_.get(); q.len[1] = mcnt_; q.op[1] = 0;
         q.a[2] = c_.get(); q.b[2] = gx_.get(); q.len[2] = n; q.op[2] = 0;
         q.a[3] = b_.get(); q.b[3] = gy_.get(); q.len[3] = mcnt_; q.op[3] = 0;
-        launch_reduce(q, part_.get(), scal_.get(), s);
-        xsum(scal_.get(), 4, RedOp::Sum);
-        hipLaunchKernelGGL(k_hsd_dphi, dim3(1), dim3(1), 0, s, scal_.get(), gamma, delta, mu, phi, psi);
-        hipLaunchKernelGGL(k_hsd_directions, dim3(kRedBlocks), dim3(NT), 0, s, m, n, scal_.get() + kIsDphi, delta, mu,
-                           fx_.get(), gx_.get(), fy_.get(), gy_.get(), x_.get(), z_.get(), y_.get(), w_.get(), D_.get(),
-                           E_.get(), dx_.get(), dz_.get(), dy_.get(), dw_.get(), part_.get());
-        hipLaunchKernelGGL(k_finish_reduce, dim3(1), dim3(kRedThreads), 0, s, part_.get(), 1, 1u, scal_.get());
-        xsum(scal_.get(), 1, RedOp::Max);
-        hipLaunchKernelGGL(k_hsd_theta, dim3(1), dim3(1), 0, s, scal_.get(), phi, psi);
-        hipLaunchKernelGGL(k_step, dim3(gv), dim3(NT), 0, s, m, n, 0.0, scal_.get() + kIsTheta, x_.get(), dx_.get(),
-                           z_.get(), dz_.get(), y_.get(), dy_.get(), w_.get(), dw_.get());
+        if (!glue || !launch_reduce_dphi(q, scal_.get(), dphi_epilogue(glue_cnt_.get(), scal_.get(), gamma, delta, mu, phi, psi), s)) {
+            launch_reduce(q, part_.get(), scal_.get(), s);
+            xsum(scal_.get(), 4, RedOp::Sum);
+            hipLaunchKernelGGL(k_hsd_dphi, dim3(1), dim3(1), 0, s, scal_.get(), gamma, delta, mu, phi, psi);
+        }
+        if (fuse_next) K.preclear(side_);
+        if (glue) {
+            hipLaunchKernelGGL(k_hsd_directions_theta, dim3(kRedBlocks), dim3(NT), 0, s, m, n, delta, mu, fx_.get(),
+                               gx_.get(), fy_.get(), gy_.get(), x_.get(), z_.get(), y_.get(), w_.get(), D_.get(),
+                               E_.get(), dx_.get(), dz_.get(), dy_.get(), dw_.get(), part_.get(), scal_.get(), phi, psi,
+                               glue_cnt_.get() + 1);
+        } else {
+            hipLaunchKernelGGL(k_hsd_directions, dim3(kRedBlocks), dim3(NT), 0, s, m, n, scal_.get() + kIsDphi, delta, mu,
+                               fx_.get(), gx_.get(), fy_.get(), gy_.get(), x_.get(), z_.get(), y_.get(), w_.get(),
+                               D_.get(), E_.get(), dx_.get(), dz_.get(), dy_.get(), dw_.get(), part_.get());
+            hipLaunchKernelGGL(k_finish_reduce, dim3(1), dim3(kRedThreads), 0, s, part_.get(), 1, 1u, scal_.get());
+            xsum(scal_.get(), 1, RedOp::Max);
+            hipLaunchKernelGGL(k_hsd_theta, dim3(1), dim3(1), 0, s, scal_.get(), phi, psi);
+        }
+        if (fuse_next) {
+            KktDevice::StepVecs sv;
+            sv.theta = scal_.get() + kIsTheta;
+            sv.x = x_.get(); sv.dx = dx_.get(); sv.z = z_.get(); sv.dz = dz_.get();
+            sv.y = y_.get(); sv.dy = dy_.get(); sv.w = w_.get(); sv.dw = dw_.get();
+            sv.E = E_.get(); sv.D = D_.get();
+            K.step_assemble(sv);
+            assembled = true;
+        } else {
+            hipLaunchKernelGGL(k_step, dim3(gv), dim3(NT), 0, s, m, n, 0.0, scal_.get() + kIsTheta, x_.get(), dx_.get(),
+                               z_.get(), dz_.get(), y_.get(), dy_.get(), w_.get(), dw_.get());
+        }
     }
     hipLaunchKernelGGL(k_unscale, dim3(gv), dim3(NT), 0, s, m, n, phi, x_.get(), z_.get(), y_.get(), w_.get());
     IPO_HIP_CHECK(hipGetLastError());
diff --git a/linear-programming-vanderbei_amd/csrc/kkt_device.h b/linear-programming-vanderbei_amd/csrc/kkt_device.h
--- a/linear-programming-vanderbei_amd/csrc/kkt_device.h
+++ b/linear-programming-vanderbei_amd/csrc/kkt_device.h
@@ -139,7 +139,17 @@
         hipStream_t stream = nullptr;
         hipEvent_t ready = nullptr;
     };
-    void factor(const double* dE, const double* dD, const PrePass* pre = nullptr);
+    void factor(const double* dE, const double* dD, const PrePass* pre = nullptr, bool assembled = false);
+
+    void preclear(hipStream_t side);
+    struct StepVecs {
+        const double* theta = nullptr;
+        double *x = nullptr, *z = nullptr, *y = nullptr, *w = nullptr;
+        const double *dx = nullptr, *dz = nullptr, *dy = nullptr, *dw = nullptr;
+        double *E = nullptr, *D = nullptr;
+    };
+    bool can_step_assemble() const { return !xch_ && qnz_ == 0; }
+    void step_assemble(const StepVecs& v);
     int solve(const double* dE, const double* dD, double* dfy, double* dfx);
     int solve2(const double* dE, const double* dD, double* dfy1, double* dfx1, double* dfy2, double* dfx2);
     void solve_multi(int R, const double* dE, const double* dD, double* const* dfy, double* const* dfx, int* ok);
@@ -187,7 +197,15 @@
     KktLaunch h_;
     PlanView plan_view() const;
     bool tail_repair() const { return use_panel_ && !xch_ && knobs_.tail_repair; }
-    void factor_core(const double* dE, const double* dD, const PrePass* pre);
+    void factor_core(const double* dE, const double* dD, const PrePass* pre, bool assembled);
+    void enqueue_clears(hipStream_t s);
+    bool preclear_pending_ = false;
+    bool assembled_ = false;
+    double asm_eps_ = 0.0;
+    bool factor_gone_ = false;
+    hipEvent_t ev_preclear_ = nullptr, ev_solve_done_ = nullptr;
+    bool solve_end_recorded_ = false;
+    DevBuf<int> dGlueCnt_;
     void dump_factor(const double* dE, const double* dD, double eps_in);
     int dump_count_ = 0;
     TailView tail_view() const;
@@ -262,7 +280,8 @@
     DevBuf<int> dfu_sup_, dfu_j_;
     DevBuf<int> dsmall_sups_;
     const bool use_panel_ = knobs_.panel;
-    bool factor_pass(const double* dE, const double* dD, bool fused, bool tail_fused, const PrePass* pre = nullptr);
+    bool factor_pass(const double* dE, const double* dD, bool fused, bool tail_fused, const PrePass* pre = nullptr,
+                     bool assembled = false);
     bool prepass_eligible(const PrePass* pre, bool fused, bool tail_fused) const;
     void enqueue_prepass(const PrePass& pre);
     void run_prepass_steps(int R, hipStream_t q);
diff --git a/linear-programming-vanderbei_amd/csrc/kkt_device.hip b/linear-programming-vanderbei_amd/csrc/kkt_device.hip
--- a/linear-programming-vanderbei_amd/csrc/kkt_device.hip
+++ b/linear-programming-vanderbei_amd/csrc/kkt_device.hip
@@ -6,6 +6,7 @@
 #include <cstdio>
 #include <cstdlib>
 #include <cstring>
+#include <stdexcept>
 
 #include "dev_common.h"
 #include "kkt_device.h"
@@ -54,6 +55,46 @@
     const int c = blockIdx.x;
     double* col = S + (size_t)c * nt;
     for (int r = (c / kPanelCols) * kPanelCols + static_cast<int>(threadIdx.x); r < nt; r += NT) col[r] = 0.0;
+}
+
+__global__ void __launch_bounds__(NT)
+k_step_assemble(int T, int m, int nbd, const int* __restrict__ perm, KktDevice::StepVecs sv, double eps,
+                const int64_t* __restrict__ dslot, double* __restrict__ Lx, int* __restrict__ live,
+                double* __restrict__ dscale, int* __restrict__ flags, int nz, const double* __restrict__ A,
+                const int64_t* __restrict__ amap) {
+    if (static_cast<int>(blockIdx.x) >= nbd) {
+        const int k = (blockIdx.x - nbd) * NT + threadIdx.x;
+        if (k < nz) Lx[amap[k]] = A[k];
+        return;
+    }
+    const int v = blockIdx.x * NT + threadIdx.x;
+    if (v < kFlagWords) flags[v] = 0;
+    if (v >= T) return;
+    const double theta = *sv.theta;
+    const int old = perm[v];
+    double a;
+    if (old < m) {
+        const int j = old;
+        const double yj = sv.y[j] + theta * sv.dy[j];
+        const double wj = sv.w[j] + theta * sv.dw[j];
+        sv.y[j] = yj;
+        sv.w[j] = wj;
+        const double e = wj / yj;
+        sv.E[j] = e;
+        a = -ref_max(e, eps);
+    } else {
+        const int i = old - m;
+        const double xi = sv.x[i] + theta * sv.dx[i];
+        const double zi = sv.z[i] + theta * sv.dz[i];
+        sv.x[i] = xi;
+        sv.z[i] = zi;
+        const double d = zi / xi;
+        sv.D[i] = d;
+        a = ref_max(d, eps);
+    }
+    Lx[dslot[v]] = a;
+    dscale[v] = fabs(a);
+    live[v] = 1;
 }
 
 typedef double double4_t __attribute__((ext_vector_type(4)));
@@ -647,15 +688,14 @@
     else *dst = *dst - v;
 }
 
-__device__ __forceinline__ void kkt_residual_body(
+__device__ __forceinline__ double kkt_residual_body(
     int m, int n, const int* __restrict__ kAt, const int* __restrict__ iAt, const double* __restrict__ At,
     const int* __restrict__ kA, const int* __restrict__ iA, const double* __restrict__ A, const double* __restrict__ E,
     const double* __restrict__ D, const double* __restrict__ fy, const double* __restrict__ fx,
     const double* __restrict__ dy, const double* __restrict__ dx, double* __restrict__ ry, double* __restrict__ rx,
-    double* __restrict__ part, int mrow, const double* __restrict__ axl, const int* __restrict__ kQ,
+    int mrow, const double* __restrict__ axl, const int* __restrict__ kQ,
     const int* __restrict__ iQ, const double* __restrict__ Q, double qmax, int qthr,
-    const double* __restrict__ qxl) {
-    __shared__ double sh[kResThreads / 64];
+    const double* __restrict__ qxl, double* sh ) {
     double mx = 0.0;
     for (int i = blockIdx.x * kResThreads + threadIdx.x; i < m + n; i += kRedBlocks * kResThreads) {
         if (i < m) {
@@ -678,8 +718,7 @@
             mx = fmax(mx, ref_abs(r));
         }
     }
-    mx = block_max_w<kResThreads / 64>(mx, sh);
-    if (threadIdx.x == 0) part[blockIdx.x] = mx;
+    return block_max_w<kResThreads / 64>(mx, sh);
 }
 
 
@@ -696,21 +735,38 @@
 __global__ void __launch_bounds__(kResThreads)
 k_kkt_residual2(int m, int n, const int* __restrict__ kAt, const int* __restrict__ iAt, const double* __restrict__ At,
                 const int* __restrict__ kA, const int* __restrict__ iA, const double* __restrict__ A,
-                const double* __restrict__ E, const double* __restrict__ D, ResJobs J, double* __restrict__ part,
+                const double* __restrict__ E, const double* __restrict__ D, ResJobs J, double* part,
                 int mrow, const int* __restrict__ kQ, const int* __restrict__ iQ, const double* __restrict__ Q,
-                double qmax, int qthr) {
+                double qmax, int qthr, PackFinish fin) {
+    __shared__ double sh[kResThreads / 64];
+    __shared__ int last;
     const int q = blockIdx.y;
-    kkt_residual_body(m, n, kAt, iAt, At, kA, iA, A, E, D, J.fy[q], J.fx[q], J.dy[q], J.dx[q], J.ry[q], J.rx[q],
-                      part + (size_t)q * kRedBlocks, mrow, J.axl[q], kQ, iQ, Q, qmax, qthr, J.qxl[q]);
+    const double mx = kkt_residual_body(m, n, kAt, iAt, At, kA, iA, A, E, D, J.fy[q], J.fx[q], J.dy[q], J.dx[q],
+                                        J.ry[q], J.rx[q], mrow, J.axl[q], kQ, iQ, Q, qmax, qthr, J.qxl[q], sh);
+    double* slot = part + (size_t)q * kRedBlocks + blockIdx.x;
+    if (!fin.cnt) {
+        if (threadIdx.x == 0) *slot = mx;
+        return;
+    }
+    if (threadIdx.x == 0) sc1_store(slot, mx);
+    if (!arrive_last(fin.cnt, static_cast<int>(gridDim.x * gridDim.y), &last)) return;
+    finish_max_pack(part, static_cast<int>(gridDim.y), fin, sh);
 }
 
 __global__ void __launch_bounds__(NT)
-k_min_abs_partial(const double* __restrict__ d, int T, double* __restrict__ part) {
+k_min_abs_partial(const double* __restrict__ d, int T, double* part, PackFinish fin) {
     __shared__ double sh[4];
+    __shared__ int last;
     double mn = HUGE_VAL;
     for (int i = blockIdx.x * NT + threadIdx.x; i < T; i += kRedBlocks * NT) mn = fmin(mn, ref_abs(d[i]));
     const double r = block_max(-mn, sh);
-    if (threadIdx.x == 0) part[blockIdx.x] = r;
+    if (!fin.cnt) {
+        if (threadIdx.x == 0) part[blockIdx.x] = r;
+        return;
+    }
+    if (threadIdx.x == 0) sc1_store(part + blockIdx.x, r);
+    if (!arrive_last(fin.cnt, kRedBlocks, &last)) return;
+    finish_max_pack(part, 1, fin, sh);
 }
 
 struct CopyOut {
@@ -989,6 +1045,10 @@
     IPO_HIP_CHECK(hipEventCreateWithFlags(&ev_pre_fork_, hipEventDisableTiming));
     IPO_HIP_CHECK(hipEventCreateWithFlags(&ev_pre_done_, hipEventDisableTiming));
     IPO_HIP_CHECK(hipEventCreateWithFlags(&ev_run_reset_, hipEventDisableTiming));
+    IPO_HIP_CHECK(hipEventCreateWithFlags(&ev_preclear_, hipEventDisableTiming));
+    IPO_HIP_CHECK(hipEventCreateWithFlags(&ev_solve_done_, hipEventDisableTiming));
+    dGlueCnt_.alloc(2);
+    IPO_HIP_CHECK(hipMemsetAsync(dGlueCnt_.get(), 0, dGlueCnt_.bytes(), s));
     IPO_HIP_CHECK(hipStreamSynchronize(s));
 }
 
@@ -1057,6 +1117,8 @@
     if (ev_pre_fork_) (void)hipEventDestroy(ev_pre_fork_);
     if (ev_pre_done_) (void)hipEventDestroy(ev_pre_done_);
     if (ev_run_reset_) (void)hipEventDestroy(ev_run_reset_);
+    if (ev_preclear_) (void)hipEventDestroy(ev_preclear_);
+    if (ev_solve_done_) (void)hipEventDestroy(ev_solve_done_);
     for (hipEvent_t e : kev_) (void)hipEventDestroy(e);
 }
 
@@ -1126,11 +1188,54 @@
     std::fclose(f);
 }
 
-void KktDevice::factor(const double* dE, const double* dD, const PrePass* pre) {
+void KktDevice::enqueue_clears(hipStream_t s) {
+    if (plan_.nt > 0 && !xch_) {
+        if (plan_.off_tail > 0) IPO_HIP_CHECK(hipMemsetAsync(dLx_.get(), 0, plan_.off_tail * sizeof(double), s));
+        hipLaunchKernelGGL(k_zero_tail_lower, dim3(plan_.nt), dim3(NT), 0, s, dLx_.get() + plan_.off_tail, plan_.nt);
+    } else {
+        IPO_HIP_CHECK(hipMemsetAsync(dLx_.get(), 0, dLx_.bytes(), s));
+    }
+}
+
+void KktDevice::preclear(hipStream_t side) {
+    if (timing_ || !side || side == stream_ || preclear_pending_) return;
+    if (!solve_end_recorded_) IPO_HIP_CHECK(hipEventRecord(ev_solve_done_, stream_));
+    IPO_HIP_CHECK(hipStreamWaitEvent(side, ev_solve_done_, 0));
+    enqueue_clears(side);
+    IPO_HIP_CHECK(hipEventRecord(ev_preclear_, side));
+    preclear_pending_ = true;
+    assembled_ = false;
+    factor_gone_ = true;
+}
+
+void KktDevice::step_assemble(const StepVecs& v) {
+    if (!can_step_assemble()) throw std::logic_error("step_assemble: not with an Exchange or a Q block");
+    hipStream_t s = stream_;
+    if (preclear_pending_) {
+        IPO_HIP_CHECK(hipStreamWaitEvent(s, ev_preclear_, 0));
+        preclear_pending_ = false;
+    } else {
+        enqueue_clears(s);
+    }
+    factor_gone_ = true;
+    const int nz = static_cast<int>(plan_.amap.size());
+    const int nbd = std::max(1, ceil_div(T_, NT));
+    hipLaunchKernelGGL(k_step_assemble, dim3(nbd + ceil_div(nz, NT)), dim3(NT), 0, s, T_, m_, nbd, dperm_.get(), v,
+                       epsdiag_, ddslot_.get(), dLx_.get(), dLive_.get(), dDscale_.get(), dFlags_.get(), nz, dA_.get(),
+                       damap_.get());
+    IPO_HIP_CHECK(hipGetLastError());
+    assembled_ = true;
+    asm_eps_ = epsdiag_;
+}
+
+void KktDevice::factor(const double* dE, const double* dD, const PrePass* pre, bool assembled) {
     const double eps_in = epsdiag_;
     drop_prepass();
+    assembled = assembled && assembled_ && asm_eps_ == epsdiag_;
+    assembled_ = false;
+    solve_end_recorded_ = false;
     try {
-        factor_core(dE, dD, pre);
+        factor_core(dE, dD, pre, assembled);
     } catch (...) {
         if (pre_state_ != kPreNone) (void)hipStreamWaitEvent(stream_, ev_pre_done_, 0);
         drop_prepass();
@@ -1139,9 +1244,10 @@
     dump_factor(dE, dD, eps_in);
 }
 
-void KktDevice::factor_core(const double* dE, const double* dD, const PrePass* pre) {
+void KktDevice::factor_core(const double* dE, const double* dD, const PrePass* pre, bool assembled) {
     const bool repair = tail_repair();
-    const bool ok = factor_pass(dE, dD, use_panel_, use_panel_, pre);
+    const bool ok = factor_pass(dE, dD, use_panel_, use_panel_, pre, assembled);
+    factor_gone_ = false;
     if (!ok) {
         tm_.panel_redos++;
         for (int b = 0; b < 4; b++) tm_.redo_where[b] += (verdict_.bail >> b) & 1;
@@ -1160,25 +1266,30 @@
     if (knobs_.epsdiag_max > 0.0 && epsdiag_ > knobs_.epsdiag_max) epsdiag_ = knobs_.epsdiag_max;
 }
 
-bool KktDevice::factor_pass(const double* dE, const double* dD, bool fused, bool tail_fused, const PrePass* pre) {
+bool KktDevice::factor_pass(const double* dE, const double* dD, bool fused, bool tail_fused, const PrePass* pre,
+                            bool assembled) {
     hipStream_t s = stream_;
     if (timing_) IPO_HIP_CHECK(hipEventRecord(ev0_, s));
     const PlanView pv = plan_view();
     const int nz = static_cast<int>(plan_.amap.size());
-    if (plan_.nt > 0 && !xch_) {
-        if (plan_.off_tail > 0) IPO_HIP_CHECK(hipMemsetAsync(dLx_.get(), 0, plan_.off_tail * sizeof(double), s));
-        hipLaunchKernelGGL(k_zero_tail_lower, dim3(plan_.nt), dim3(NT), 0, s, dLx_.get() + plan_.off_tail, plan_.nt);
-    } else {
-        IPO_HIP_CHECK(hipMemsetAsync(dLx_.get(), 0, dLx_.bytes(), s));
-    }
-    if (nz > 0) hipLaunchKernelGGL(k_assemble_A, dim3(ceil_div(nz, NT)), dim3(NT), 0, s, nz, dA_.get(), damap_.get(), dLx_.get());
-    if (qnz_ > 0)
-        hipLaunchKernelGGL(k_assemble_Q, dim3(ceil_div(qnz_, NT)), dim3(NT), 0, s, qnz_, dQ_.get(), dqmap_.get(),
-                           static_cast<double>(qmax_), dLx_.get());
-    hipLaunchKernelGGL(k_assemble_diag, dim3(ceil_div(T_, NT)), dim3(NT), 0, s, T_, m_, dperm_.get(), dE, dD, epsdiag_,
-                       ddslot_.get(), dLx_.get(), dLive_.get(), dDscale_.get(), shard_minor() ? plan_.tail_c0 : T_,
-                       dFlags_.get(), dkQ_.get() ? dQdiag_.get() : static_cast<const double*>(nullptr),
-                       static_cast<double>(qmax_));
+    if (preclear_pending_) {
+        IPO_HIP_CHECK(hipStreamWaitEvent(s, ev_preclear_, 0));
+        preclear_pending_ = false;
+    } else if (!assembled) {
+        enqueue_clears(s);
+    }
+    if (!assembled) {
+        if (nz > 0)
+            hipLaunchKernelGGL(k_assemble_A, dim3(ceil_div(nz, NT)), dim3(NT), 0, s, nz, dA_.get(), damap_.get(),
+                               dLx_.get());
+        if (qnz_ > 0)
+            hipLaunchKernelGGL(k_assemble_Q, dim3(ceil_div(qnz_, NT)), dim3(NT), 0, s, qnz_, dQ_.get(), dqmap_.get(),
+                               static_cast<double>(qmax_), dLx_.get());
+        hipLaunchKernelGGL(k_assemble_diag, dim3(ceil_div(T_, NT)), dim3(NT), 0, s, T_, m_, dperm_.get(), dE, dD,
+                           epsdiag_, ddslot_.get(), dLx_.get(), dLive_.get(), dDscale_.get(),
+                           shard_minor() ? plan_.tail_c0 : T_, dFlags_.get(),
+                           dkQ_.get() ? dQdiag_.get() : static_cast<const double*>(nullptr), static_cast<double>(qmax_));
+    }
     const TailView tv = tail_view();
     if (!prepass_eligible(pre, fused, tail_fused)) pre = nullptr;
     enqueue_levels(pv, tv, fused, s, pre);
@@ -1300,8 +1411,17 @@
 bool KktDevice::finish_pass(bool fused) {
     hipStream_t s = stream_;
     IPO_HIP_CHECK(hipGetLastError());
-    hipLaunchKernelGGL(k_min_abs_partial, dim3(kRedBlocks), dim3(NT), 0, s, dDg_.get(), T_, dPart_.get());
-    if (xch_) {
+    PackFinish fin;
+    if (!xch_ && knobs_.glue) {
+        fin.cnt = dGlueCnt_.get();
+        fin.out = dFacScal_.get() + kFsNegMinD;
+        fin.f = dFlags_.get();
+        fin.nf = kFlagReadWords;
+        fin.outi = dFacScal_.get() + kFsFlags;
+    }
+    hipLaunchKernelGGL(k_min_abs_partial, dim3(kRedBlocks), dim3(NT), 0, s, dDg_.get(), T_, dPart_.get(), fin);
+    if (fin.cnt) {
+    } else if (xch_) {
         static_assert(kFsNegMinD == 0 && kFsNdepMax == 1 && kFsBailMax == 2, "one allreduce over the three");
         hipLaunchKernelGGL(k_finish_reduce, dim3(1), dim3(kRedThreads), 0, s, dPart_.get(), 1, 1u,
                            dFacScal_.get() + kFsNegMinD);
@@ -1526,6 +1646,7 @@
     hipStream_t s = stream_;
     if (timing_) IPO_HIP_CHECK(hipEventRecord(ev0_, s));
     const int m = m_, n = n_, T = T_;
+    if (factor_gone_ && R > 0) throw std::logic_error("solve: no factorisation since the factor storage was cleared");
     const bool pre_lead = pre_lead_;
     const bool pre = take_prepass(R, dfy, dfx);
     if (!pre && R > 0) enqueue_pass_head(R, dfy, dfx, dPart_.get(), s);
@@ -1559,6 +1680,14 @@
         else rawsolve(zv(active[0] ? 0 : 1), 1, fwd_first);
         eps_cleared_ = false;
         int nq = 0;
+        PackFinish fin;
+        if (!xch_ && knobs_.glue) {
+            fin.cnt = dGlueCnt_.get() + 1;
+            fin.out = dScal_.get() + kScRes;
+            fin.f = dIncons_.get();
+            fin.nf = 2;
+            fin.outi = dScal_.get() + kScIncons;
+        }
         {
             PermJobs P{};
             ResJobs J{};
@@ -1587,9 +1716,10 @@
             hipLaunchKernelGGL(k_kkt_residual2, dim3(kRedBlocks, nq), dim3(kResThreads), 0, s, m, n, dkAt_.get(),
                                diAt_.get(), dAt_.get(), dkA_.get(), diA_.get(), dA_.get(), dE, dD, J, dPart_.get(), mrow,
                                dkQ_.get() ? dkQ_.get() : static_cast<const int*>(nullptr), diQ_.get(), dQ_.get(),
-                               static_cast<double>(qmax_), q_long_min());
-        }
-        if (xch_) {
+                               static_cast<double>(qmax_), q_long_min(), fin);
+        }
+        if (fin.cnt) {
+        } else if (xch_) {
             hipLaunchKernelGGL(k_finish_reduce, dim3(1), dim3(kRedThreads), 0, s, dPart_.get(), nq, (1u << nq) - 1u,
                                dScal_.get() + kScRes);
             xsum(dScal_.get() + kScRes, nq, RedOp::Max);
@@ -1632,6 +1762,10 @@
     co.n = n;
     co.R = R;
     if (R > 0 && m + n > 0) hipLaunchKernelGGL(k_copy_out, dim3(ceil_div(R * (m + n), NT)), dim3(NT), 0, s, co);
+    if (knobs_.glue && !xch_ && !timing_) {
+        IPO_HIP_CHECK(hipEventRecord(ev_solve_done_, s));
+        solve_end_recorded_ = true;
+    }
     if (timing_) {
         IPO_HIP_CHECK(hipEventRecord(ev1_, s));
         IPO_HIP_CHECK(hipStreamSynchronize(s));
diff --git a/linear-programming-vanderbei_amd/csrc/kkt_kernels.h b/linear-programming-vanderbei_amd/csrc/kkt_kernels.h
--- a/linear-programming-vanderbei_amd/csrc/kkt_kernels.h
+++ b/linear-programming-vanderbei_amd/csrc/kkt_kernels.h
@@ -4,6 +4,7 @@
 #include <cstdint>
 #include <vector>
 
+#include "dev_common.h"
 #include "kkt_device.h"
 #include "kkt_plan.h"
 
@@ -46,15 +47,6 @@
     return (x < r ? x * (q + 1) : r * (q + 1) + (x - r) * q) + i;
 }
 
-static __device__ __forceinline__ void sc1_store(double* p, double v) {
-    __hip_atomic_store(p, v, __ATOMIC_RELAXED, __HIP_MEMORY_SCOPE_AGENT);
-}
-static __device__ __forceinline__ double sc1_load(const double* p) {
-    return __hip_atomic_load(const_cast<double*>(p), __ATOMIC_RELAXED, __HIP_MEMORY_SCOPE_AGENT);
-}
-static __device__ __forceinline__ int sc1_load_int(const int* p) {
-    return __hip_atomic_load(const_cast<int*>(p), __ATOMIC_RELAXED, __HIP_MEMORY_SCOPE_AGENT);
-}
 template <bool SC>
 static __device__ __forceinline__ double ld_h(const double* p) {
     if constexpr (SC) return sc1_load(p);
diff --git a/linear-programming-vanderbei_amd/csrc/kkt_knobs.h b/linear-programming-vanderbei_amd/csrc/kkt_knobs.h
--- a/linear-programming-vanderbei_amd/csrc/kkt_knobs.h
+++ b/linear-programming-vanderbei_amd/csrc/kkt_knobs.h
@@ -20,6 +20,7 @@
     bool sf = true;
     bool overlap = true;
     bool prepass = true;
+    bool glue = true;
     int lead_trail = -1;
     int lead_trail_mode(int ntb) const { return lead_trail >= 0 ? lead_trail : ntb >= kTrailMinBlocks ? 2 : 0; }
     int lead_helpers = kTrailHelpers;
@@ -87,6 +88,7 @@
         k.sf = flag("IPO_HIP_SF", true);
         k.overlap = flag("IPO_HIP_OVERLAP", true);
         k.prepass = flag("IPO_HIP_PREPASS", true);
+        k.glue = flag("IPO_HIP_GLUE", true);
         k.lead_trail = num("IPO_HIP_LEAD_TRAIL", -1);
         if (k.lead_trail < 0 || k.lead_trail > 2) k.lead_trail = -1;
         k.lead_helpers = std::max(1, num("IPO_HIP_LEAD_HELPERS", kTrailHelpers));
diff --git a/linear-programming-vanderbei_amd/csrc/kkt_sweep.hip b/linear-programming-vanderbei_amd/csrc/kkt_sweep.hip
--- a/linear-programming-vanderbei_amd/csrc/kkt_sweep.hip
+++ b/linear-programming-vanderbei_amd/csrc/kkt_sweep.hip
@@ -2221,6 +2221,7 @@
 
 void KktDevice::rawsolve(double* dz, int R, size_t fwd_first) {
     hipStream_t s = stream_;
+    solve_end_recorded_ = false;
     double* epsp = sweep_eps();
     if (ndep_ > 0) {
         RedJobs j{};
```

Result: no change. 320.3 iterations/s, median of 6 (+0.8%).
